# facebookresearch/metamorph

Measured on AMD Instinct MI355X. Metric: train tokens/sec (LLaMA-3-8B + SigLIP-SO400M, seq2048, 256 img toks), whole job, higher is better.
Workload: dtype bf16

## Files before the change

metamorph_amd/csrc/attn.hip:

```cpp
#include "mm355_common.h"
#include "attn2.h"
#include <cstdlib>
#include <algorithm>

namespace {

constexpr int NT = 256;

__global__ __launch_bounds__(NT) void attn_delta_kernel(const uint16_t* __restrict__ o, const uint16_t* __restrict__ d_o, int64_t ld_o,
                                                        float* __restrict__ delta, int L, int Hq, int d) {
    const int l = blockIdx.x * 64 + (threadIdx.x >> 2), part = threadIdx.x & 3;
    const int h = blockIdx.y, b = blockIdx.z;
    const int dv = d >> 3;
    float s = 0.f;
    if (l < L) {
        for (int v = part; v < dv; v += 4) {
            float x[8], y[8];
            unpack8(*(const u32x4*)(o + ((int64_t)b * L + l) * ld_o + (int64_t)h * d + v * 8), x);
            unpack8(*(const u32x4*)(d_o + ((int64_t)b * L + l) * ld_o + (int64_t)h * d + v * 8), y);
#pragma unroll
            for (int e = 0; e < 8; ++e) s += x[e] * y[e];
        }
    }
    s += __shfl_xor(s, 1, 64);
    s += __shfl_xor(s, 2, 64);
    if (part == 0 && l < L) delta[((int64_t)b * Hq + h) * L + l] = s;
}

__global__ __launch_bounds__(NT) void group_reduce_kernel(const float* __restrict__ part, uint16_t* __restrict__ out, int64_t ld_out, int64_t rows,
                                                          int Hq, int Hkv, int d) {
    const int group = Hq / Hkv, cv = (Hkv * d) >> 3;
    const int64_t total = rows * cv;
    for (int64_t i = blockIdx.x * (int64_t)NT + threadIdx.x; i < total; i += (int64_t)gridDim.x * NT) {
        const int64_t r = i / cv; const int c = (int)(i % cv) * 8;
        const int hk = c / d, cc = c % d;
        float acc[8] = {0.f, 0.f, 0.f, 0.f, 0.f, 0.f, 0.f, 0.f};
        for (int g = 0; g < group; ++g) {
            const float* p = part + r * ((int64_t)Hq * d) + (int64_t)(hk * group + g) * d + cc;
            const f32x4 x0 = *(const f32x4*)p, x1 = *(const f32x4*)(p + 4);
            acc[0] += x0.x; acc[1] += x0.y; acc[2] += x0.z; acc[3] += x0.w;
            acc[4] += x1.x; acc[5] += x1.y; acc[6] += x1.z; acc[7] += x1.w;
        }
        *(u32x4*)(out + r * ld_out + c) = pack8(acc);
    }
}

int pick_dp(int64_t d) { return d <= 64 ? 64 : (d <= 96 ? 96 : 128); }

bool bad_geom(int64_t B, int64_t L, int64_t Hq, int64_t Hkv, int64_t d) {
    return B <= 0 || L <= 0 || Hq <= 0 || Hkv <= 0 || (Hq % Hkv) || d <= 0 || d > 128 || (d & 7) || L > 0x7fffffff;
}

bool fast128(int64_t d, int64_t ld_k) { return d == 128 && ld_k * 2 * 64 < 0x7fffffff; }

}

namespace {
int attn_fwd_impl(const mm355_bf16* q, const mm355_bf16* k, const mm355_bf16* v, int64_t ld_q, int64_t ld_k, mm355_bf16* o,
                  int64_t ld_o, float* lse, const int32_t* seqlens, int64_t B, int64_t L, int64_t Hq, int64_t Hkv,
                  int64_t d, float scale, int causal, int variant, void* stream, int32_t* dbg = nullptr) {
    (void)hipGetLastError();
    if (!q || !k || !v || !o || !lse || bad_geom(B, L, Hq, Hkv, d)) return MM355_EINVAL;
    if ((ld_q & 7) || (ld_k & 7) || (ld_o & 7)) return MM355_EINVAL;
    attn2::Args a{q, k, v, nullptr, ld_q, ld_k, ld_o, o, lse, nullptr, nullptr, nullptr, 0, seqlens,
                  nullptr, nullptr, nullptr, nullptr, 0, (int)B, (int)L, (int)Hq, (int)Hkv, (int)d, scale, causal, nullptr, nullptr, nullptr, dbg};
    const bool can4 = d == 128 && L * ld_k * 2 < 0x7fffffffll;
    if (variant == 4 || variant == 41) return can4 ? mm355_attn4_fwd_launch(a, variant == 41, (hipStream_t)stream) : MM355_EUNSUPPORTED;
    if (variant == 3) return MM355_EUNSUPPORTED;
    if (variant == 2) return mm355_attn2_fwd_launch(a, pick_dp(d), (hipStream_t)stream);
    if (variant != 0) return MM355_EINVAL;
    if (can4 && fast128(d, ld_k)) return mm355_attn4_fwd_launch(a, 0, (hipStream_t)stream);
    return mm355_attn2_fwd_launch(a, pick_dp(d), (hipStream_t)stream);
}
}

extern "C" int mm355_attn_fwd(const mm355_bf16* q, const mm355_bf16* k, const mm355_bf16* v, int64_t ld_q, int64_t ld_k, mm355_bf16* o,
                              int64_t ld_o, float* lse, const int32_t* seqlens, int64_t B, int64_t L, int64_t Hq, int64_t Hkv,
                              int64_t d, float scale, int causal, void* stream) {
    return attn_fwd_impl(q, k, v, ld_q, ld_k, o, ld_o, lse, seqlens, B, L, Hq, Hkv, d, scale, causal, 0, stream);
}

extern "C" int mm355_attn_fwd_variant(const mm355_bf16* q, const mm355_bf16* k, const mm355_bf16* v, int64_t ld_q, int64_t ld_k, mm355_bf16* o,
                                      int64_t ld_o, float* lse, const int32_t* seqlens, int64_t B, int64_t L, int64_t Hq, int64_t Hkv,
                                      int64_t d, float scale, int causal, int variant, void* stream) {
    return attn_fwd_impl(q, k, v, ld_q, ld_k, o, ld_o, lse, seqlens, B, L, Hq, Hkv, d, scale, causal, variant, stream);
}

extern "C" int mm355_attn_fwd_debug(const mm355_bf16* q, const mm355_bf16* k, const mm355_bf16* v, int64_t ld_q, int64_t ld_k, mm355_bf16* o,
                                    int64_t ld_o, float* lse, const int32_t* seqlens, int64_t B, int64_t L, int64_t Hq, int64_t Hkv,
                                    int64_t d, float scale, int causal, int variant, int32_t* rescale_counts, void* stream) {
    if (!rescale_counts || (variant != 4 && variant != 41)) return MM355_EINVAL;
    return attn_fwd_impl(q, k, v, ld_q, ld_k, o, ld_o, lse, seqlens, B, L, Hq, Hkv, d, scale, causal, variant, stream, rescale_counts);
}

extern "C" int mm355_attn_bwd_prep(const mm355_bf16* o, const mm355_bf16* d_o, int64_t ld_o, float* delta, int64_t B, int64_t L,
                                   int64_t Hq, int64_t d, void* stream) {
    (void)hipGetLastError();
    if (!o || !d_o || !delta || B <= 0 || L <= 0 || Hq <= 0 || d <= 0 || d > 128 || (d & 7) || (ld_o & 7)) return MM355_EINVAL;
    dim3 grid((unsigned)((L + 63) / 64), (unsigned)Hq, (unsigned)B);
    hipLaunchKernelGGL(attn_delta_kernel, grid, dim3(NT), 0, (hipStream_t)stream, o, d_o, ld_o, delta, (int)L, (int)Hq, (int)d);
    return mm_launch_status();
}

extern "C" int64_t mm355_attn_bwd_ws_floats(int64_t B, int64_t L, int64_t Hq, int64_t Hkv, int64_t d, int64_t ld_max) {
    if (fast128(d, ld_max)) return 2 * B * Hq * L;
    if (Hq == Hkv) return 0;
    return 2 * B * L * Hq * d;
}

namespace {
int attn_bwd_impl(const mm355_bf16* q, const mm355_bf16* k, const mm355_bf16* v, int64_t ld_q, int64_t ld_k, const mm355_bf16* d_o,
                  int64_t ld_o, const float* lse, const float* delta, const int32_t* seqlens, mm355_bf16* dq, int64_t ld_dq,
                  mm355_bf16* dk, mm355_bf16* dv, int64_t ld_dkv, int64_t B, int64_t L, int64_t Hq, int64_t Hkv, int64_t d,
                  float scale, int causal, float* workspace, const uint16_t* rope_cos, const uint16_t* rope_sin, const int32_t* rope_pos,
                  int variant, void* stream) {
    (void)hipGetLastError();
    if (!q || !k || !v || !d_o || !lse || !delta || !dq || !dk || !dv || bad_geom(B, L, Hq, Hkv, d)) return MM355_EINVAL;
    if ((ld_q & 7) || (ld_k & 7) || (ld_o & 7) || (ld_dkv & 7) || (ld_dq & 7)) return MM355_EINVAL;
    const int64_t ld_max = std::max(std::max(ld_q, ld_k), ld_o);
    if (variant == 3) return MM355_EUNSUPPORTED;
    if (variant != 0 && variant != 2 && variant != 4 && variant != 41) return MM355_EINVAL;
    const bool is128 = fast128(d, ld_max) && variant != 2;
    const bool can4 = is128 && workspace && L * ld_max * 2 < 0x7fffffffll;
    if (is128 && !can4 && Hq != Hkv) return workspace ? MM355_EUNSUPPORTED : MM355_EINVAL;
    if (rope_cos && !can4) return MM355_EUNSUPPORTED;
    if ((variant == 4 || variant == 41) && !can4) return MM355_EUNSUPPORTED;
    if (variant == 4 || variant == 41 || (variant == 0 && can4)) {
        attn2::Args a4{q, k, v, d_o, ld_q, ld_k, ld_o, nullptr, nullptr, lse, delta, dq, ld_dq, seqlens,
                       dk, dv, nullptr, nullptr, ld_dkv, (int)B, (int)L, (int)Hq, (int)Hkv, (int)d, scale, causal, rope_cos, rope_sin, rope_pos};
        return mm355_attn4_bwd_launch(a4, workspace, variant == 41, (hipStream_t)stream);
    }
    if (Hq != Hkv && !workspace) return MM355_EINVAL;
    hipStream_t s = (hipStream_t)stream;
    float* dkp = nullptr;
    float* dvp = nullptr;
    if (Hq != Hkv) {
        dkp = workspace;
        dvp = workspace + (int64_t)B * L * Hq * d;
    }
    attn2::Args a{q, k, v, d_o, ld_q, ld_k, ld_o, nullptr, nullptr, lse, delta, dq, ld_dq, seqlens,
                  dk, dv, dkp, dvp, ld_dkv, (int)B, (int)L, (int)Hq, (int)Hkv, (int)d, scale, causal, rope_cos, rope_sin, rope_pos};
    int rc = mm355_attn2_dkdv_launch(a, pick_dp(d), s);
    if (rc != MM355_OK) return rc;
    if (dkp) {
        const int64_t rows = B * L;
        const unsigned rg = (unsigned)std::min<int64_t>((rows * (Hkv * d / 8) + NT - 1) / NT, 4096);
        hipLaunchKernelGGL(group_reduce_kernel, dim3(rg), dim3(NT), 0, s, dkp, dk, ld_dkv, rows, (int)Hq, (int)Hkv, (int)d);
        hipLaunchKernelGGL(group_reduce_kernel, dim3(rg), dim3(NT), 0, s, dvp, dv, ld_dkv, rows, (int)Hq, (int)Hkv, (int)d);
        rc = mm_launch_status();
        if (rc != MM355_OK) return rc;
    }
    return mm355_attn2_dq_launch(a, pick_dp(d), s);
}
}

extern "C" int mm355_attn_bwd(const mm355_bf16* q, const mm355_bf16* k, const mm355_bf16* v, int64_t ld_q, int64_t ld_k, const mm355_bf16* d_o,
                              int64_t ld_o, const float* lse, const float* delta, const int32_t* seqlens, mm355_bf16* dq, int64_t ld_dq,
                              mm355_bf16* dk, mm355_bf16* dv, int64_t ld_dkv, int64_t B, int64_t L, int64_t Hq, int64_t Hkv, int64_t d,
                              float scale, int causal, float* workspace, void* stream) {
    return attn_bwd_impl(q, k, v, ld_q, ld_k, d_o, ld_o, lse, delta, seqlens, dq, ld_dq, dk, dv, ld_dkv, B, L, Hq, Hkv, d, scale, causal, workspace,
                         nullptr, nullptr, nullptr, 0, stream);
}

extern "C" int mm355_attn_bwd_rope(const mm355_bf16* q, const mm355_bf16* k, const mm355_bf16* v, int64_t ld_q, int64_t ld_k, const mm355_bf16* d_o,
                                   int64_t ld_o, const float* lse, const float* delta, const int32_t* seqlens, mm355_bf16* dq, int64_t ld_dq,
                                   mm355_bf16* dk, mm355_bf16* dv, int64_t ld_dkv, int64_t B, int64_t L, int64_t Hq, int64_t Hkv, int64_t d,
                                   float scale, int causal, const mm355_bf16* cos_t, const mm355_bf16* sin_t, const int32_t* pos_offset,
                                   float* workspace, void* stream) {
    if (!cos_t || !sin_t) return MM355_EINVAL;
    return attn_bwd_impl(q, k, v, ld_q, ld_k, d_o, ld_o, lse, delta, seqlens, dq, ld_dq, dk, dv, ld_dkv, B, L, Hq, Hkv, d, scale, causal, workspace,
                         cos_t, sin_t, pos_offset, 0, stream);
}

extern "C" int mm355_attn_bwd_variant(const mm355_bf16* q, const mm355_bf16* k, const mm355_bf16* v, int64_t ld_q, int64_t ld_k, const mm355_bf16* d_o,
                                      int64_t ld_o, const float* lse, const float* delta, const int32_t* seqlens, mm355_bf16* dq, int64_t ld_dq,
                                      mm355_bf16* dk, mm355_bf16* dv, int64_t ld_dkv, int64_t B, int64_t L, int64_t Hq, int64_t Hkv, int64_t d,
                                      float scale, int causal, const mm355_bf16* cos_t, const mm355_bf16* sin_t, const int32_t* pos_offset,
                                      float* workspace, int variant, void* stream) {
    if ((cos_t == nullptr) != (sin_t == nullptr)) return MM355_EINVAL;
    return attn_bwd_impl(q, k, v, ld_q, ld_k, d_o, ld_o, lse, delta, seqlens, dq, ld_dq, dk, dv, ld_dkv, B, L, Hq, Hkv, d, scale, causal, workspace,
                         cos_t, sin_t, pos_offset, variant, stream);
}
```

metamorph_amd/csrc/attn4.hip:

```cpp
#include "attn2.h"

#ifndef ATTN4_GEN_DIR
#define ATTN4_GEN_DIR attn4_gen
#endif
#define ATTN4_STR2(x) #x
#define ATTN4_STR(x) ATTN4_STR2(x)
#define ATTN4_INC(f) ATTN4_STR(ATTN4_GEN_DIR/f)

namespace attn4 {
using namespace attn2;

constexpr int TILE = 16384;
constexpr int VRING = 2 * TILE;
constexpr float LOG2E = 1.4426950408889634f;
constexpr float THR = 6.0f;

MM_DEV float half_swap_max(float m) {
    float a = m, b = m;
    asm volatile("" : "+v"(b));
    swap32(a, b);
    return max2_raw(a, b);
}
MM_DEV float half_swap_sum(float m) {
    float a = m, b = m;
    asm volatile("" : "+v"(b));
    swap32(a, b);
    return a + b;
}

#define ATTN4_BARRIER() do { if (do_bar) asm volatile("s_waitcnt vmcnt(0)\n\ts_barrier" ::: "memory"); } while (0)
#define ATTN4_DMA_K(i) do { __builtin_amdgcn_sched_barrier(0); \
    __builtin_amdgcn_raw_ptr_buffer_load_lds(rsK, (lptr_t)(smem + kdst + (i) * 1024), 16, kvo[i], 0, 0, 0); __builtin_amdgcn_sched_barrier(0); } while (0)
#define ATTN4_DMA_V(i) do { if (do_bar) { __builtin_amdgcn_sched_barrier(0); \
    __builtin_amdgcn_raw_ptr_buffer_load_lds(rsV, (lptr_t)(smem + vdst + (i) * 1024), 16, vvo[i], 0, 0, 0); __builtin_amdgcn_sched_barrier(0); } } while (0)
template <bool SAFE>
__global__ __launch_bounds__(256, 1) __attribute__((amdgpu_num_vgpr(64))) void fwd_kernel(Args a) {
    __shared__ __attribute__((aligned(16))) unsigned char smem[4 * TILE];
    asm volatile("" ::: "v255", "a255");
#ifdef MM355_ATTN4_TIMING
    const long long tm0 = __builtin_readcyclecounter();
    long long tm1 = 0, tm2 = 0, tm3 = 0, tm4 = 0, tm5 = 0;
#define ATTN4_STAMP(x) x = __builtin_readcyclecounter()
#else
#define ATTN4_STAMP(x) do {} while (0)
#endif
    const int tid = threadIdx.x, lane = tid & 63;
    const int wave = __builtin_amdgcn_readfirstlane(tid >> 6);
    const int c = lane & 31, hi = lane >> 5;
    int xb, hq, b;
    block_coords((a.L + 255) / 256, a.Hq, inner_heads(a.Hq, a.Hq / a.Hkv), true, xb, hq, b);
    const int q0 = xb * 256;
    const int hk = hq / (a.Hq / a.Hkv);
    const int L = a.L;
    const int seqlen = a.seqlens ? min(a.seqlens[b], L) : L;
    const int64_t row_base = (int64_t)b * L;
    uint16_t* o_base = a.o + row_base * a.ld_o + (int64_t)hq * 128;
    float* lse_base = a.lse + ((int64_t)b * a.Hq + hq) * L;

    if (q0 >= seqlen) {
        for (int v = tid; v < 256 * 16; v += 256) {
            const int r = v >> 4, cc = (v & 15) * 8;
            if (q0 + r < L) *(u32x4*)(o_base + (int64_t)(q0 + r) * a.ld_o + cc) = u32x4{0u, 0u, 0u, 0u};
        }
        if (q0 + tid < L) lse_base[q0 + tid] = 0.f;
        return;
    }
    const int kv_end = a.causal ? min(seqlen, q0 + 256) : seqlen;
    const int T = (kv_end + 63) >> 6;
    const int qw0 = q0 + wave * 64;
    const int tw = qw0 < seqlen ? (a.causal ? min(T - 1, min(qw0 + 63, seqlen - 1) >> 6) : T - 1) : -1;

    const uint32_t ldb = (uint32_t)a.ld_k * 2u;
    const uint16_t* kbase = a.k + row_base * a.ld_k + (int64_t)hk * 128;
    const uint16_t* vbase = a.v + row_base * a.ld_k + (int64_t)hk * 128;
    const uint32_t nrec = (uint32_t)(seqlen - 1) * ldb + 256u;
    __amdgpu_buffer_rsrc_t rsK, rsV;
#define ATTN4_TILE_RSRC(base_, tile_) __builtin_amdgcn_make_buffer_rsrc((void*)((base_) + (int64_t)(tile_) * 64 * a.ld_k), 0, \
    (tile_) < T ? nrec - (uint32_t)(tile_) * 64u * ldb : 0u, 0x00020000)
    uint32_t kvo[4], vvo[4];
    {
        const int r4 = lane >> 4, pc = lane & 15;
#pragma unroll
        for (int i = 0; i < 4; ++i) {
            const uint32_t row = 16 * wave + 4 * i + r4;
            kvo[i] = row * ldb + (uint32_t)((pc ^ (4 * i + r4)) << 4);
            vvo[i] = row * ldb + (uint32_t)((pc ^ (r4 << 2)) << 4);
        }
    }
    const float sl2 = a.scale * LOG2E;
    const uint32_t sl2b_ = __builtin_amdgcn_readfirstlane(__float_as_uint(sl2));
    {
        const uint16_t* qp0_ = a.q + (row_base + min(qw0 + c, L - 1)) * a.ld_q + (int64_t)hq * 128 + hi * 8;
        const uint16_t* qp1_ = a.q + (row_base + min(qw0 + 32 + c, L - 1)) * a.ld_q + (int64_t)hq * 128 + hi * 8;
#include ATTN4_INC(q_load.inc)
    }
    bool do_bar = true;
    int kdst, vdst;
    rsK = ATTN4_TILE_RSRC(kbase, 0); rsV = ATTN4_TILE_RSRC(vbase, 0); kdst = wave * 4096; vdst = VRING + wave * 4096;
#pragma unroll
    for (int i = 0; i < 4; ++i) { ATTN4_DMA_K(i); }
#pragma unroll
    for (int i = 0; i < 4; ++i) { ATTN4_DMA_V(i); }
    rsK = ATTN4_TILE_RSRC(kbase, 1); kdst = TILE + wave * 4096;
#pragma unroll
    for (int i = 0; i < 4; ++i) { ATTN4_DMA_K(i); }
#include ATTN4_INC(zero_o.inc)
    float LS[2][4] = {{0.f, 0.f, 0.f, 0.f}, {0.f, 0.f, 0.f, 0.f}};
    float MX[2][2], rm_[2], rt_[2];
    uint64_t grow_ = 0;
    int nresc_ = 0;
#define ATTN4_COUNT_RESCALE() (++nresc_)
    float thr_ = THR / sl2;
    asm volatile("" : "+v"(thr_));
    const float ninf = -INFINITY;
    int KA[8], VA[4];
#pragma unroll
    for (int ks = 0; ks < 8; ++ks) KA[ks] = c * 256 + (((ks * 2 + hi) ^ (c & 15)) << 4);
    {
        const int g = lane >> 4, i = lane & 15;
#pragma unroll
        for (int db = 0; db < 4; ++db)
            VA[db] = VRING + (4 * hi + (i >> 2)) * 256 + ((((db * 4 + (g & 1) * 2 + ((i & 3) >> 1)) ^ ((i >> 2) << 2))) << 4) + (i & 1) * 8;
    }
#pragma unroll
    for (int ks = 0; ks < 8; ++ks) asm volatile("" : "+v"(KA[ks]));
#pragma unroll
    for (int i = 0; i < 4; ++i) { asm volatile("" : "+v"(VA[i])); asm volatile("" : "+v"(kvo[i])); asm volatile("" : "+v"(vvo[i])); }
    int lim2[2] = {0, 0};
    if (tw >= 0) {
#pragma unroll
        for (int qb = 0; qb < 2; ++qb) {
            const int qg = qw0 + qb * 32 + c;
            lim2[qb] = (a.causal ? min(qg, seqlen - 1) : seqlen - 1) - tw * 64 - 4 * hi;
        }
    }
    asm volatile("s_waitcnt vmcnt(12)" ::: "memory");
#include ATTN4_INC(q_pre01.inc)
    asm volatile("s_waitcnt vmcnt(0)" ::: "memory");
    __builtin_amdgcn_s_barrier();

#define ATTN4_STEP_VARS(s_) do { const int s__ = (s_); \
    rsK = ATTN4_TILE_RSRC(kbase, s__ + 2); rsV = ATTN4_TILE_RSRC(vbase, s__ + 2); \
    kdst = (s__ & 1) * TILE + wave * 4096; vdst = VRING + (s__ & 1) * TILE + wave * 4096; } while (0)

    ATTN4_STAMP(tm1);
    if (tw >= 0) {
        bool mask_next = tw == 0;
        ATTN4_STEP_VARS(-1);
        if constexpr (SAFE) {
#include ATTN4_INC(safe_head.inc)
        } else {
#include ATTN4_INC(head.inc)
        }
        ATTN4_STAMP(tm2);
        int t = 0;
        for (;;) {
            if (t >= tw) break;
            mask_next = t + 1 == tw;
            ATTN4_STEP_VARS(t);
            if constexpr (SAFE) {
#include ATTN4_INC(safe_loop0.inc)
            } else {
#include ATTN4_INC(loop0.inc)
            }
            ++t;
            if (t >= tw) break;
            mask_next = t + 1 == tw;
            ATTN4_STEP_VARS(t);
            if constexpr (SAFE) {
#include ATTN4_INC(safe_loop1.inc)
            } else {
#include ATTN4_INC(loop1.inc)
            }
            ++t;
        }
        ATTN4_STAMP(tm3);
        do_bar = tw <= T - 2;
        ATTN4_STEP_VARS(tw);
        if (tw & 1) {
            if constexpr (SAFE) {
#include ATTN4_INC(safe_tail1.inc)
            } else {
#include ATTN4_INC(tail1.inc)
            }
        } else {
            if constexpr (SAFE) {
#include ATTN4_INC(safe_tail0.inc)
            } else {
#include ATTN4_INC(tail0.inc)
            }
        }
    }
    ATTN4_STAMP(tm4);
    do_bar = true;
    for (int s = tw < 0 ? -1 : tw + 1; s <= T - 2; ++s) {
        ATTN4_STEP_VARS(s);
        if (s >= 0) {
#pragma unroll
            for (int i = 0; i < 4; ++i) { ATTN4_DMA_K(i); }
        }
        ATTN4_BARRIER();
#pragma unroll
        for (int i = 0; i < 4; ++i) { ATTN4_DMA_V(i); }
    }
    asm volatile("s_nop 15\n\ts_nop 15\n\ts_nop 15\n\ts_nop 15\n\ts_waitcnt vmcnt(0) lgkmcnt(0)" ::: "memory");
    __syncthreads();
    ATTN4_STAMP(tm5);

    unsigned char* so = smem + wave * TILE;
#pragma unroll
    for (int qb_ = 0; qb_ < 2; ++qb_) {
        const int qg = qw0 + qb_ * 32 + c;
        const bool valid = qg < seqlen && tw >= 0;
        const float l_run = half_swap_sum((LS[qb_][0] + LS[qb_][1]) + (LS[qb_][2] + LS[qb_][3]));
        const float inv = (valid && l_run > 0.f) ? 1.0f / l_run : 0.f;
#pragma unroll
        for (int db_ = 0; db_ < 4; ++db_) {
            float x_[16];
#include ATTN4_INC(epi_read.inc)
#pragma unroll
            for (int i4 = 0; i4 < 4; ++i4) {
                u32x2 w;
                w.x = pack2bf(x_[4 * i4 + 0] * inv, x_[4 * i4 + 1] * inv);
                w.y = pack2bf(x_[4 * i4 + 2] * inv, x_[4 * i4 + 3] * inv);
                *(u32x2*)(so + (qb_ * 32 + c) * 256 + (((db_ * 4 + i4) ^ (c & 15)) << 4) + hi * 8) = w;
            }
        }
        float nm0;
        if (qb_ == 0) asm volatile("v_mov_b32 %0, v192" : "=v"(nm0)); else asm volatile("v_mov_b32 %0, v208" : "=v"(nm0));
        if (hi == 0 && qg < L) lse_base[qg] = valid ? (log2f(l_run) - nm0 * sl2) * 0.6931471805599453f : 0.f;
    }
    __syncthreads();
#pragma unroll
    for (int k = 0; k < 16; ++k) {
        const int r = 4 * k + (lane >> 4), j = lane & 15;
        const int qg = qw0 + r;
        if (qg < L) *(u32x4*)(o_base + (int64_t)qg * a.ld_o + j * 8) = *(const u32x4*)(so + r * 256 + ((j ^ (r & 15)) << 4));
    }
    if (a.dbg && lane == 0) a.dbg[(((int64_t)b * a.Hq + hq) * ((L + 255) / 256) + xb) * 4 + wave] = nresc_;
#ifdef MM355_ATTN4_TIMING
    asm volatile("s_waitcnt vmcnt(0)" ::: "memory");
    const long long tm6 = __builtin_readcyclecounter();
    if (lane == 0 && (wave == 0 || wave == 3) && q0 + 64 <= L) {
        long long* w = (long long*)(lse_base + q0) + (wave == 3 ? 8 : 0);
        w[0] = tm1 - tm0; w[1] = tm2 - tm1; w[2] = tm3 - tm2; w[3] = tm4 - tm3; w[4] = tm5 - tm4; w[5] = tm6 - tm5; w[6] = tw; w[7] = T;
    }
#endif
}

}

int mm355_attn4_fwd_launch(const attn2::Args& a, int variant, hipStream_t s) {
    const int64_t nblk = (int64_t)((a.L + 255) / 256) * a.Hq * a.B;
    if (nblk > 0x7fffffff) return MM355_EINVAL;
    if (variant == 1) hipLaunchKernelGGL(attn4::fwd_kernel<true>, dim3((unsigned)nblk), dim3(256), 0, s, a);
    else hipLaunchKernelGGL(attn4::fwd_kernel<false>, dim3((unsigned)nblk), dim3(256), 0, s, a);
    return mm_launch_status();
}
```

metamorph_amd/csrc/attn4_bwd.hip:

```cpp
#include "attn2.h"

#ifndef ATTN4B_GEN_DIR
#define ATTN4B_GEN_DIR attn4_bwd_gen
#endif
#define ATTN4B_STR2(x) #x
#define ATTN4B_STR(x) ATTN4B_STR2(x)
#define ATTN4B_INC(f) ATTN4B_STR(ATTN4B_GEN_DIR/f)

namespace attn4b {
using namespace attn2;

constexpr float LOG2E = 1.4426950408889634f;
constexpr int SLOT = 32768;
constexpr int KV_BASE = 2048;
constexpr int KV_LDS = KV_BASE + 4 * SLOT, Q_LDS = 4 * SLOT;

MM_DEV int rot4(int row) { return ((row & 3) << 2) | ((row >> 2) & 3); }

struct LaneAddr {
    int RA[8], TA[4], TB[4], SA;
    MM_DEV void init(int lane) {
        const int c = lane & 31, hi = lane >> 5, g = lane >> 4, i = lane & 15;
#pragma unroll
        for (int ks = 0; ks < 8; ++ks) RA[ks] = c * 256 + (((ks * 2 + hi) ^ rot4(c)) << 4);
        const int row0 = 4 * hi + (i >> 2), row1 = row0 + 8;
#pragma unroll
        for (int db = 0; db < 4; ++db) {
            const int chunk = db * 4 + (g & 1) * 2 + ((i & 3) >> 1);
            TA[db] = row0 * 256 + ((chunk ^ rot4(row0)) << 4) + (i & 1) * 8;
            TB[db] = row1 * 256 + ((chunk ^ rot4(row1)) << 4) + (i & 1) * 8;
        }
        SA = hi * 16;
    }
};
MM_DEV void piece_offsets(int wave, int lane, uint32_t ldb, uint32_t (&vo)[4]) {
    const int r4 = lane >> 4, pc = lane & 15;
#pragma unroll
    for (int i = 0; i < 4; ++i) vo[i] = (uint32_t)(16 * wave + 4 * i + r4) * ldb + (uint32_t)((pc ^ ((r4 << 2) | i)) << 4);
}
MM_DEV uint32_t scale_pair(uint32_t w, float s) { return pack2bf(bflo(w) * s, bfhi(w) * s); }

#define BWD_BARRIER() asm volatile("s_waitcnt vmcnt(%0)\n\ts_barrier" :: "n"(NDMA) : "memory")

template <bool SAFE>
__global__ __launch_bounds__(256, 1) __attribute__((amdgpu_num_vgpr(96))) void dkdv_kernel(Args a, const float* __restrict__ nstat) {
    extern __shared__ __attribute__((aligned(16))) unsigned char smem[];
    asm volatile("" ::: "v255", "a255");
#ifdef MM355_ATTN4_TIMING
    const long long tm0 = __builtin_readcyclecounter();
    long long tm1 = 0, tm2 = 0, tm3 = 0, tm4 = 0;
#define BWD_STAMP(x) x = __builtin_readcyclecounter()
#else
#define BWD_STAMP(x) do {} while (0)
#endif
    constexpr int NDMA = 9;
    const int tid = threadIdx.x, lane = tid & 63;
    const int wave = __builtin_amdgcn_readfirstlane(tid >> 6);
    const int c = lane & 31, hi = lane >> 5;
    const int rep = a.Hq / a.Hkv;
    int xb, hk, b;
    block_coords((a.L + 127) / 128, a.Hkv, inner_heads(a.Hkv, 1), false, xb, hk, b);
    const int kv0 = xb * 128;
    const int L = a.L;
    const int seqlen = a.seqlens ? min(a.seqlens[b], L) : L;
    const int64_t row_base = (int64_t)b * L;
    const int kw0 = kv0 + 32 * wave;

    if (kv0 >= seqlen) {
        for (int v = tid; v < 128 * 16; v += 256) {
            const int r = v >> 4, cc = (v & 15) * 8;
            if (kv0 + r < L) {
                *(u32x4*)(a.dk + (row_base + kv0 + r) * a.ld_dkv + (int64_t)hk * 128 + cc) = u32x4{0u, 0u, 0u, 0u};
                *(u32x4*)(a.dv + (row_base + kv0 + r) * a.ld_dkv + (int64_t)hk * 128 + cc) = u32x4{0u, 0u, 0u, 0u};
            }
        }
        return;
    }
    const int q_start = a.causal ? kv0 : 0;
    const int n_it = (seqlen - q_start + 63) >> 6;
    const int n_tot = n_it * rep;
    const uint32_t ldqb = (uint32_t)a.ld_q * 2u, ldob = (uint32_t)a.ld_o * 2u;
    const int64_t stat_n = (int64_t)a.B * a.Hq * L;

    const uint32_t sl2b_ = __builtin_amdgcn_readfirstlane(__float_as_uint(a.scale * LOG2E));
    LaneAddr la;
    la.init(lane);
    int RA[8], TA[4], TB[4], RAH[8], TAH[4], TBH[4], SA = la.SA;
#pragma unroll
    for (int i = 0; i < 8; ++i) { RA[i] = la.RA[i] + KV_BASE; RAH[i] = RA[i] + 65536; asm volatile("" : "+v"(RA[i])); asm volatile("" : "+v"(RAH[i])); }
#pragma unroll
    for (int i = 0; i < 4; ++i) {
        TA[i] = la.TA[i] + KV_BASE; TB[i] = la.TB[i] + KV_BASE; TAH[i] = TA[i] + 65536; TBH[i] = TB[i] + 65536;
        asm volatile("" : "+v"(TA[i])); asm volatile("" : "+v"(TB[i])); asm volatile("" : "+v"(TAH[i])); asm volatile("" : "+v"(TBH[i]));
    }
    asm volatile("" : "+v"(SA));
    uint32_t qvo[4], ovo[4], svo = (uint32_t)lane * 4u;
    piece_offsets(wave, lane, ldqb, qvo);
    piece_offsets(wave, lane, ldob, ovo);
#pragma unroll
    for (int i = 0; i < 4; ++i) { asm volatile("" : "+v"(qvo[i])); asm volatile("" : "+v"(ovo[i])); }
    asm volatile("" : "+v"(svo));
    const float ninf = -INFINITY;
    float t0_;
    const int kg = kw0 + c;
    const int qmin = kg >= seqlen ? seqlen : (a.causal ? kg : 0);
    const int mlo_base = qmin - 4 * hi;
    const unsigned mspan_ = (unsigned)(seqlen - qmin);
    int mlo_ = 0;
    bool mask_cur = false;

    __amdgpu_buffer_rsrc_t rsQ, rsO, rsS;
    int dst0 = 0;
    int dg = 0, dit = 0, cg = 0, cit = 0;
#define KV_TILE_VARS(slot_) do { \
        const bool live_ = dg < rep; \
        const int qt0_ = q_start + dit * 64; \
        const int hq_ = hk * rep + dg; \
        rsQ = __builtin_amdgcn_make_buffer_rsrc((void*)(a.q + (row_base + qt0_) * a.ld_q + (int64_t)hq_ * 128), 0, live_ ? (uint32_t)(seqlen - qt0_ - 1) * ldqb + 256u : 0u, 0x00020000); \
        rsO = __builtin_amdgcn_make_buffer_rsrc((void*)(a.d_o + (row_base + qt0_) * a.ld_o + (int64_t)hq_ * 128), 0, live_ ? (uint32_t)(seqlen - qt0_ - 1) * ldob + 256u : 0u, 0x00020000); \
        rsS = __builtin_amdgcn_make_buffer_rsrc((void*)(nstat + (wave & 1) * stat_n + ((int64_t)b * a.Hq + hq_) * L + qt0_), 0, live_ ? (uint32_t)(L - qt0_) * 4u : 0u, 0x00020000); \
        dst0 = (slot_); \
        if (++dit == n_it) { dit = 0; ++dg; } } while (0)
#define BWD_DMA(i) do { __builtin_amdgcn_sched_barrier(0); \
        if ((i) < 4) __builtin_amdgcn_raw_ptr_buffer_load_lds(rsQ, (lptr_t)(smem + KV_BASE + dst0 * SLOT + (wave * 4 + (i)) * 1024), 16, qvo[(i) & 3], 0, 0, 0); \
        else if ((i) < 8) __builtin_amdgcn_raw_ptr_buffer_load_lds(rsO, (lptr_t)(smem + KV_BASE + dst0 * SLOT + 16384 + (wave * 4 + (i) - 4) * 1024), 16, ovo[(i) & 3], 0, 0, 0); \
        else __builtin_amdgcn_raw_ptr_buffer_load_lds(rsS, (lptr_t)(smem + dst0 * 512 + (wave & 1) * 256), 4, svo, 0, 0, 0); \
        __builtin_amdgcn_sched_barrier(0); } while (0)
#define KV_MASK_VARS() do { \
        const int qt0_ = q_start + cit * 64; \
        mask_cur = (a.causal && qt0_ < kw0 + 31) || qt0_ + 64 > seqlen || kw0 + 32 > seqlen; \
        mlo_ = mlo_base - qt0_; \
        if (++cit == n_it) { cit = 0; ++cg; } } while (0)

    KV_TILE_VARS(0);
#pragma unroll
    for (int i = 0; i < 9; ++i) { BWD_DMA(i); }
    KV_TILE_VARS(1);
#pragma unroll
    for (int i = 0; i < 9; ++i) { BWD_DMA(i); }
    {
        const int key = min(kw0 + c, L - 1);
        const uint16_t* p0_ = a.k + (row_base + key) * a.ld_k + (int64_t)hk * 128 + hi * 8;
        const uint16_t* p1_ = a.v + (row_base + key) * a.ld_k + (int64_t)hk * 128 + hi * 8;
#include ATTN4B_INC(kv_pers_load.inc)
    }
#include ATTN4B_INC(kv_zero.inc)
    asm volatile("s_waitcnt vmcnt(0)" ::: "memory");
    {
        float t1_;
#include ATTN4B_INC(kv_pers_place.inc)
    }
    __builtin_amdgcn_s_barrier();

    BWD_STAMP(tm1);
    KV_TILE_VARS(2);
    if constexpr (SAFE) {
#include ATTN4B_INC(kv_safe_head.inc)
    } else {
#include ATTN4B_INC(kv_head.inc)
    }
    BWD_STAMP(tm2);
    int u = 0;
    for (;;) {
        if (u >= n_tot - 1) break;
        KV_TILE_VARS(3); KV_MASK_VARS();
        if constexpr (SAFE) {
#include ATTN4B_INC(kv_safe_loop0.inc)
        } else {
#include ATTN4B_INC(kv_loop0.inc)
        }
        ++u;
        if (u >= n_tot - 1) break;
        KV_TILE_VARS(0); KV_MASK_VARS();
        if constexpr (SAFE) {
#include ATTN4B_INC(kv_safe_loop1.inc)
        } else {
#include ATTN4B_INC(kv_loop1.inc)
        }
        ++u;
        if (u >= n_tot - 1) break;
        KV_TILE_VARS(1); KV_MASK_VARS();
        if constexpr (SAFE) {
#include ATTN4B_INC(kv_safe_loop2.inc)
        } else {
#include ATTN4B_INC(kv_loop2.inc)
        }
        ++u;
        if (u >= n_tot - 1) break;
        KV_TILE_VARS(2); KV_MASK_VARS();
        if constexpr (SAFE) {
#include ATTN4B_INC(kv_safe_loop3.inc)
        } else {
#include ATTN4B_INC(kv_loop3.inc)
        }
        ++u;
    }
    BWD_STAMP(tm3);
    KV_MASK_VARS();
    switch (u & 3) {
    case 0:
        if constexpr (SAFE) {
#include ATTN4B_INC(kv_safe_tail0.inc)
        } else {
#include ATTN4B_INC(kv_tail0.inc)
        }
        break;
    case 1:
        if constexpr (SAFE) {
#include ATTN4B_INC(kv_safe_tail1.inc)
        } else {
#include ATTN4B_INC(kv_tail1.inc)
        }
        break;
    case 2:
        if constexpr (SAFE) {
#include ATTN4B_INC(kv_safe_tail2.inc)
        } else {
#include ATTN4B_INC(kv_tail2.inc)
        }
        break;
    default:
        if constexpr (SAFE) {
#include ATTN4B_INC(kv_safe_tail3.inc)
        } else {
#include ATTN4B_INC(kv_tail3.inc)
        }
        break;
    }
#undef BWD_DMA
    asm volatile("s_nop 15\n\ts_nop 15\n\ts_nop 15\n\ts_nop 15\n\ts_waitcnt vmcnt(0) lgkmcnt(0)" ::: "memory");
    __syncthreads();
    BWD_STAMP(tm4);

    unsigned char* so = smem + wave * 16384;
    const int pos = min(kg, L - 1) + (a.rope_pos ? a.rope_pos[b] : 0);
#pragma unroll
    for (int which_ = 0; which_ < 2; ++which_) {
        const float sc = which_ == 0 ? a.scale : 1.0f;
#pragma unroll
        for (int dbp = 0; dbp < 2; ++dbp)
#pragma unroll
            for (int i4_ = 0; i4_ < 4; ++i4_) {
                float x_[4], lo_[4], hi_[4];
                {
                    const int db_ = dbp;
#include ATTN4B_INC(kv_acc_read.inc)
#pragma unroll
                    for (int r = 0; r < 4; ++r) lo_[r] = x_[r] * sc;
                }
                {
                    const int db_ = dbp + 2;
#include ATTN4B_INC(kv_acc_read.inc)
#pragma unroll
                    for (int r = 0; r < 4; ++r) hi_[r] = x_[r] * sc;
                }
                if (which_ == 0 && a.rope_cos) {
                    const int col = dbp * 32 + 8 * i4_ + 4 * hi;
                    const u32x2 cw = *(const u32x2*)(a.rope_cos + (int64_t)pos * 128 + col);
                    const u32x2 sw = *(const u32x2*)(a.rope_sin + (int64_t)pos * 128 + col);
                    const float cs[4] = {bflo(cw.x), bfhi(cw.x), bflo(cw.y), bfhi(cw.y)};
                    const float sn[4] = {bflo(sw.x), bfhi(sw.x), bflo(sw.y), bfhi(sw.y)};
#pragma unroll
                    for (int r = 0; r < 4; ++r) {
                        const float x1 = round_bf(lo_[r]), x2 = round_bf(hi_[r]);
                        lo_[r] = x1 * cs[r] + x2 * sn[r];
                        hi_[r] = x2 * cs[r] - x1 * sn[r];
                    }
                }
#pragma unroll
                for (int half = 0; half < 2; ++half) {
                    const int db = dbp + 2 * half;
                    const float* s4 = half ? hi_ : lo_;
                    u32x2 w;
                    w.x = pack2bf(s4[0], s4[1]);
                    w.y = pack2bf(s4[2], s4[3]);
                    *(u32x2*)(so + which_ * 8192 + c * 256 + (((db * 4 + i4_) ^ (c & 15)) << 4) + hi * 8) = w;
                }
            }
    }
    __syncthreads();
#pragma unroll
    for (int which_ = 0; which_ < 2; ++which_)
#pragma unroll
        for (int k = 0; k < 8; ++k) {
            const int r = 4 * k + (lane >> 4), j = lane & 15;
            const int key = kw0 + r;
            if (key < L) {
                u32x4 val = *(const u32x4*)(so + which_ * 8192 + r * 256 + ((j ^ (r & 15)) << 4));
                if (key >= seqlen) val = u32x4{0u, 0u, 0u, 0u};
                *(u32x4*)((which_ ? a.dv : a.dk) + (row_base + key) * a.ld_dkv + (int64_t)hk * 128 + j * 8) = val;
            }
        }
#ifdef MM355_ATTN4_TIMING
    asm volatile("s_waitcnt vmcnt(0)" ::: "memory");
    const long long tm5 = __builtin_readcyclecounter();
    __syncthreads();
    if (tid == 0) {
        long long* w = (long long*)(a.dk + (row_base + kv0) * a.ld_dkv + (int64_t)hk * 128);
        w[0] = tm1 - tm0; w[1] = tm2 - tm1; w[2] = tm3 - tm2; w[3] = tm4 - tm3; w[4] = tm5 - tm4; w[5] = n_tot;
    }
#endif
}

template <bool SAFE>
__global__ __launch_bounds__(256, 1) __attribute__((amdgpu_num_vgpr(80))) void dq_kernel(Args a) {
    extern __shared__ __attribute__((aligned(16))) unsigned char smem[];
    asm volatile("" ::: "v255", "a255");
    constexpr int NDMA = 8;
    const int tid = threadIdx.x, lane = tid & 63;
    const int wave = __builtin_amdgcn_readfirstlane(tid >> 6);
    const int c = lane & 31, hi = lane >> 5;
    int xb, hq, b;
    block_coords((a.L + 127) / 128, a.Hq, inner_heads(a.Hq, a.Hq / a.Hkv), true, xb, hq, b);
    const int q0 = xb * 128;
    const int hk = hq / (a.Hq / a.Hkv);
    const int L = a.L;
    const int seqlen = a.seqlens ? min(a.seqlens[b], L) : L;
    const int64_t row_base = (int64_t)b * L;
    uint16_t* dq_base = a.dqb + row_base * a.ld_dq + (int64_t)hq * 128;
    if (q0 >= seqlen) {
        for (int v = tid; v < 128 * 16; v += 256) {
            const int r = v >> 4, cc = (v & 15) * 8;
            if (q0 + r < L) *(u32x4*)(dq_base + (int64_t)(q0 + r) * a.ld_dq + cc) = u32x4{0u, 0u, 0u, 0u};
        }
        return;
    }
    const int kv_end = a.causal ? min(seqlen, q0 + 128) : seqlen;
    const int n_tot = (kv_end + 63) >> 6;
    const int qw0 = q0 + 32 * wave;
    const int qg = qw0 + c;
    const uint32_t ldb = (uint32_t)a.ld_k * 2u;
    const uint16_t* kbase = a.k + row_base * a.ld_k + (int64_t)hk * 128;
    const uint16_t* vbase = a.v + row_base * a.ld_k + (int64_t)hk * 128;
    const uint32_t nrec = (uint32_t)(seqlen - 1) * ldb + 256u;

    const uint32_t sl2b_ = __builtin_amdgcn_readfirstlane(__float_as_uint(a.scale * LOG2E));
    LaneAddr la;
    la.init(lane);
    int RA[8], TA[4], TB[4], RAH[8], TAH[4], TBH[4];
#pragma unroll
    for (int i = 0; i < 8; ++i) { RA[i] = la.RA[i]; RAH[i] = RA[i] + 65536; asm volatile("" : "+v"(RA[i])); asm volatile("" : "+v"(RAH[i])); }
#pragma unroll
    for (int i = 0; i < 4; ++i) {
        TA[i] = la.TA[i]; TB[i] = la.TB[i]; TAH[i] = TA[i] + 65536; TBH[i] = TB[i] + 65536;
        asm volatile("" : "+v"(TA[i])); asm volatile("" : "+v"(TB[i])); asm volatile("" : "+v"(TAH[i])); asm volatile("" : "+v"(TBH[i]));
    }
    uint32_t kvo[4];
    piece_offsets(wave, lane, ldb, kvo);
#pragma unroll
    for (int i = 0; i < 4; ++i) asm volatile("" : "+v"(kvo[i]));
    const float ninf = -INFINITY;
    const int kmax = qg >= seqlen ? -1 : (a.causal ? min(qg, seqlen - 1) : seqlen - 1);
    const int mlim_base = kmax - 4 * hi;
    int mlim_ = 0;
    bool mask_cur = false;

    __amdgpu_buffer_rsrc_t rsK, rsV;
    int dst0 = 0, dt = 0, ct = 0;
#define Q_TILE_VARS(slot_) do { \
        rsK = __builtin_amdgcn_make_buffer_rsrc((void*)(kbase + (int64_t)dt * 64 * a.ld_k), 0, dt < n_tot ? nrec - (uint32_t)dt * 64u * ldb : 0u, 0x00020000); \
        rsV = __builtin_amdgcn_make_buffer_rsrc((void*)(vbase + (int64_t)dt * 64 * a.ld_k), 0, dt < n_tot ? nrec - (uint32_t)dt * 64u * ldb : 0u, 0x00020000); \
        dst0 = (slot_) * SLOT; ++dt; } while (0)
#define BWD_DMA(i) do { __builtin_amdgcn_sched_barrier(0); \
        if ((i) < 4) __builtin_amdgcn_raw_ptr_buffer_load_lds(rsK, (lptr_t)(smem + dst0 + (wave * 4 + (i)) * 1024), 16, kvo[(i) & 3], 0, 0, 0); \
        else __builtin_amdgcn_raw_ptr_buffer_load_lds(rsV, (lptr_t)(smem + dst0 + 16384 + (wave * 4 + (i) - 4) * 1024), 16, kvo[(i) & 3], 0, 0, 0); \
        __builtin_amdgcn_sched_barrier(0); } while (0)
#define Q_MASK_VARS() do { \
        const int kt0_ = ct * 64; \
        mask_cur = (a.causal && kt0_ + 63 > qw0) || kt0_ + 64 > seqlen || qw0 + 32 > seqlen; \
        mlim_ = mlim_base - kt0_; ++ct; } while (0)

    Q_TILE_VARS(0);
#pragma unroll
    for (int i = 0; i < 8; ++i) { BWD_DMA(i); }
    Q_TILE_VARS(1);
#pragma unroll
    for (int i = 0; i < 8; ++i) { BWD_DMA(i); }
    {
        const int qc = min(qg, L - 1);
        const uint16_t* p0_ = a.q + (row_base + qc) * a.ld_q + (int64_t)hq * 128 + hi * 8;
        const uint16_t* p1_ = a.d_o + (row_base + qc) * a.ld_o + (int64_t)hq * 128 + hi * 8;
#include ATTN4B_INC(q_pers_load.inc)
        const float nl_ = -a.lse_in[((int64_t)b * a.Hq + hq) * L + qc] * (1.0f / a.scale);
        const float nd_ = -a.delta[((int64_t)b * a.Hq + hq) * L + qc];
#include ATTN4B_INC(q_tuple_write.inc)
    }
#include ATTN4B_INC(q_zero.inc)
    asm volatile("s_waitcnt vmcnt(0)" ::: "memory");
    {
        float t0_, t1_;
#include ATTN4B_INC(q_pers_place.inc)
    }
    __builtin_amdgcn_s_barrier();

    Q_TILE_VARS(2);
    if constexpr (SAFE) {
#include ATTN4B_INC(q_safe_head.inc)
    } else {
#include ATTN4B_INC(q_head.inc)
    }
    int u = 0;
    for (;;) {
        if (u >= n_tot - 1) break;
        Q_TILE_VARS(3); Q_MASK_VARS();
        if constexpr (SAFE) {
#include ATTN4B_INC(q_safe_loop0.inc)
        } else {
#include ATTN4B_INC(q_loop0.inc)
        }
        ++u;
        if (u >= n_tot - 1) break;
        Q_TILE_VARS(0); Q_MASK_VARS();
        if constexpr (SAFE) {
#include ATTN4B_INC(q_safe_loop1.inc)
        } else {
#include ATTN4B_INC(q_loop1.inc)
        }
        ++u;
        if (u >= n_tot - 1) break;
        Q_TILE_VARS(1); Q_MASK_VARS();
        if constexpr (SAFE) {
#include ATTN4B_INC(q_safe_loop2.inc)
        } else {
#include ATTN4B_INC(q_loop2.inc)
        }
        ++u;
        if (u >= n_tot - 1) break;
        Q_TILE_VARS(2); Q_MASK_VARS();
        if constexpr (SAFE) {
#include ATTN4B_INC(q_safe_loop3.inc)
        } else {
#include ATTN4B_INC(q_loop3.inc)
        }
        ++u;
    }
    Q_MASK_VARS();
    switch (u & 3) {
    case 0:
        if constexpr (SAFE) {
#include ATTN4B_INC(q_safe_tail0.inc)
        } else {
#include ATTN4B_INC(q_tail0.inc)
        }
        break;
    case 1:
        if constexpr (SAFE) {
#include ATTN4B_INC(q_safe_tail1.inc)
        } else {
#include ATTN4B_INC(q_tail1.inc)
        }
        break;
    case 2:
        if constexpr (SAFE) {
#include ATTN4B_INC(q_safe_tail2.inc)
        } else {
#include ATTN4B_INC(q_tail2.inc)
        }
        break;
    default:
        if constexpr (SAFE) {
#include ATTN4B_INC(q_safe_tail3.inc)
        } else {
#include ATTN4B_INC(q_tail3.inc)
        }
        break;
    }
#undef BWD_DMA
    asm volatile("s_nop 15\n\ts_nop 15\n\ts_nop 15\n\ts_nop 15\n\ts_waitcnt vmcnt(0) lgkmcnt(0)" ::: "memory");
    __syncthreads();

    unsigned char* so = smem + wave * 8192;
    const float keep = qg < seqlen ? a.scale : 0.0f;
    const int pos = min(qg, L - 1) + (a.rope_pos ? a.rope_pos[b] : 0);
#pragma unroll
    for (int dbp = 0; dbp < 2; ++dbp)
#pragma unroll
        for (int i4_ = 0; i4_ < 4; ++i4_) {
            constexpr int which_ = 0;
            float x_[4], lo_[4], hi_[4];
            {
                const int db_ = dbp;
#include ATTN4B_INC(q_acc_read.inc)
#pragma unroll
                for (int r = 0; r < 4; ++r) lo_[r] = x_[r] * keep;
            }
            {
                const int db_ = dbp + 2;
#include ATTN4B_INC(q_acc_read.inc)
#pragma unroll
                for (int r = 0; r < 4; ++r) hi_[r] = x_[r] * keep;
            }
            if (a.rope_cos) {
                const int col = dbp * 32 + 8 * i4_ + 4 * hi;
                const u32x2 cw = *(const u32x2*)(a.rope_cos + (int64_t)pos * 128 + col);
                const u32x2 sw = *(const u32x2*)(a.rope_sin + (int64_t)pos * 128 + col);
                const float cs[4] = {bflo(cw.x), bfhi(cw.x), bflo(cw.y), bfhi(cw.y)};
                const float sn[4] = {bflo(sw.x), bfhi(sw.x), bflo(sw.y), bfhi(sw.y)};
#pragma unroll
                for (int r = 0; r < 4; ++r) {
                    const float x1 = round_bf(lo_[r]), x2 = round_bf(hi_[r]);
                    lo_[r] = x1 * cs[r] + x2 * sn[r];
                    hi_[r] = x2 * cs[r] - x1 * sn[r];
                }
            }
#pragma unroll
            for (int half = 0; half < 2; ++half) {
                const int db = dbp + 2 * half;
                const float* s4 = half ? hi_ : lo_;
                u32x2 w;
                w.x = pack2bf(s4[0], s4[1]);
                w.y = pack2bf(s4[2], s4[3]);
                *(u32x2*)(so + c * 256 + (((db * 4 + i4_) ^ (c & 15)) << 4) + hi * 8) = w;
            }
        }
    __syncthreads();
#pragma unroll
    for (int k = 0; k < 8; ++k) {
        const int r = 4 * k + (lane >> 4), j = lane & 15;
        if (qw0 + r < L) *(u32x4*)(dq_base + (int64_t)(qw0 + r) * a.ld_dq + j * 8) = *(const u32x4*)(so + r * 256 + ((j ^ (r & 15)) << 4));
    }
}

__global__ __launch_bounds__(256) void nstat_kernel(const float* __restrict__ lse, const float* __restrict__ delta, float* __restrict__ nstat, int64_t n,
                                                    float inv_scale) {
    for (int64_t i = blockIdx.x * 256ll + threadIdx.x; i < n; i += (int64_t)gridDim.x * 256) {
        nstat[i] = -lse[i] * inv_scale;
        nstat[n + i] = -delta[i];
    }
}

}

int mm355_attn4_bwd_launch(const attn2::Args& a, float* workspace, int variant, hipStream_t s) {
    static std::atomic<uint64_t> ok_kv{0}, ok_kvs{0}, ok_q{0}, ok_qs{0};
    const int64_t n = (int64_t)a.B * a.Hq * a.L;
    hipLaunchKernelGGL(attn4b::nstat_kernel, dim3((unsigned)std::min<int64_t>((n + 255) / 256, 2048)), dim3(256), 0, s, a.lse_in, a.delta, workspace, n, 1.0f / a.scale);
    const int64_t nkv = (int64_t)((a.L + 127) / 128) * a.Hkv * a.B, nq = (int64_t)((a.L + 127) / 128) * a.Hq * a.B;
    if (nkv > 0x7fffffff || nq > 0x7fffffff) return MM355_EINVAL;
    if (variant == 1) {
        if (mm_ensure_dynamic_lds((const void*)attn4b::dkdv_kernel<true>, attn4b::KV_LDS, ok_kvs) != MM355_OK) return MM355_ELAUNCH;
        if (mm_ensure_dynamic_lds((const void*)attn4b::dq_kernel<true>, attn4b::Q_LDS, ok_qs) != MM355_OK) return MM355_ELAUNCH;
        hipLaunchKernelGGL(attn4b::dkdv_kernel<true>, dim3((unsigned)nkv), dim3(256), attn4b::KV_LDS, s, a, (const float*)workspace);
        hipLaunchKernelGGL(attn4b::dq_kernel<true>, dim3((unsigned)nq), dim3(256), attn4b::Q_LDS, s, a);
    } else {
        if (mm_ensure_dynamic_lds((const void*)attn4b::dkdv_kernel<false>, attn4b::KV_LDS, ok_kv) != MM355_OK) return MM355_ELAUNCH;
        if (mm_ensure_dynamic_lds((const void*)attn4b::dq_kernel<false>, attn4b::Q_LDS, ok_q) != MM355_OK) return MM355_ELAUNCH;
        hipLaunchKernelGGL(attn4b::dkdv_kernel<false>, dim3((unsigned)nkv), dim3(256), attn4b::KV_LDS, s, a, (const float*)workspace);
        hipLaunchKernelGGL(attn4b::dq_kernel<false>, dim3((unsigned)nq), dim3(256), attn4b::Q_LDS, s, a);
    }
    return mm_launch_status();
}
```

Baseline: 25740.

## Pair causal query blocks per workgroup in attn4 forward and dq kernels

For causal attention, each workgroup in the attn4 forward and dq-backward kernels now handles two query blocks, a late one and an early one (nb-1-xb and xb). This balances the triangular workload across workgroups and halves the grid. It also prefetches the next block's Q and K/V while the current block's epilogue runs, using a larger dynamic LDS region so the output staging buffer is separate. New variant codes (41-45) select the pairing and safe modes. The cost is a more complex kernel with more register pressure and extra LDS.

Result: no change. 25650 (-0.3%).

```diff
diff --git a/metamorph_amd/csrc/attn.hip b/metamorph_amd/csrc/attn.hip
--- a/metamorph_amd/csrc/attn.hip
+++ b/metamorph_amd/csrc/attn.hip
@@ -53,6 +53,8 @@
 
 bool fast128(int64_t d, int64_t ld_k) { return d == 128 && ld_k * 2 * 64 < 0x7fffffff; }
 
+int stream_variant(int variant) { return variant == 4 ? 0 : (variant >= 41 && variant <= 45 ? variant - 40 : -1); }
+
 }
 
 namespace {
@@ -65,7 +67,7 @@
     attn2::Args a{q, k, v, nullptr, ld_q, ld_k, ld_o, o, lse, nullptr, nullptr, nullptr, 0, seqlens,
                   nullptr, nullptr, nullptr, nullptr, 0, (int)B, (int)L, (int)Hq, (int)Hkv, (int)d, scale, causal, nullptr, nullptr, nullptr, dbg};
     const bool can4 = d == 128 && L * ld_k * 2 < 0x7fffffffll;
-    if (variant == 4 || variant == 41) return can4 ? mm355_attn4_fwd_launch(a, variant == 41, (hipStream_t)stream) : MM355_EUNSUPPORTED;
+    if (stream_variant(variant) >= 0) return can4 ? mm355_attn4_fwd_launch(a, stream_variant(variant), (hipStream_t)stream) : MM355_EUNSUPPORTED;
     if (variant == 3) return MM355_EUNSUPPORTED;
     if (variant == 2) return mm355_attn2_fwd_launch(a, pick_dp(d), (hipStream_t)stream);
     if (variant != 0) return MM355_EINVAL;
@@ -89,7 +91,7 @@
 extern "C" int mm355_attn_fwd_debug(const mm355_bf16* q, const mm355_bf16* k, const mm355_bf16* v, int64_t ld_q, int64_t ld_k, mm355_bf16* o,
                                     int64_t ld_o, float* lse, const int32_t* seqlens, int64_t B, int64_t L, int64_t Hq, int64_t Hkv,
                                     int64_t d, float scale, int causal, int variant, int32_t* rescale_counts, void* stream) {
-    if (!rescale_counts || (variant != 4 && variant != 41)) return MM355_EINVAL;
+    if (!rescale_counts || stream_variant(variant) < 0) return MM355_EINVAL;
     return attn_fwd_impl(q, k, v, ld_q, ld_k, o, ld_o, lse, seqlens, B, L, Hq, Hkv, d, scale, causal, variant, stream, rescale_counts);
 }
 
@@ -119,16 +121,17 @@
     if ((ld_q & 7) || (ld_k & 7) || (ld_o & 7) || (ld_dkv & 7) || (ld_dq & 7)) return MM355_EINVAL;
     const int64_t ld_max = std::max(std::max(ld_q, ld_k), ld_o);
     if (variant == 3) return MM355_EUNSUPPORTED;
-    if (variant != 0 && variant != 2 && variant != 4 && variant != 41) return MM355_EINVAL;
+    const int sv = stream_variant(variant);
+    if (variant != 0 && variant != 2 && sv < 0) return MM355_EINVAL;
     const bool is128 = fast128(d, ld_max) && variant != 2;
     const bool can4 = is128 && workspace && L * ld_max * 2 < 0x7fffffffll;
     if (is128 && !can4 && Hq != Hkv) return workspace ? MM355_EUNSUPPORTED : MM355_EINVAL;
     if (rope_cos && !can4) return MM355_EUNSUPPORTED;
-    if ((variant == 4 || variant == 41) && !can4) return MM355_EUNSUPPORTED;
-    if (variant == 4 || variant == 41 || (variant == 0 && can4)) {
+    if (sv >= 0 && !can4) return MM355_EUNSUPPORTED;
+    if (sv >= 0 || (variant == 0 && can4)) {
         attn2::Args a4{q, k, v, d_o, ld_q, ld_k, ld_o, nullptr, nullptr, lse, delta, dq, ld_dq, seqlens,
                        dk, dv, nullptr, nullptr, ld_dkv, (int)B, (int)L, (int)Hq, (int)Hkv, (int)d, scale, causal, rope_cos, rope_sin, rope_pos};
-        return mm355_attn4_bwd_launch(a4, workspace, variant == 41, (hipStream_t)stream);
+        return mm355_attn4_bwd_launch(a4, workspace, sv >= 0 ? sv : 0, (hipStream_t)stream);
     }
     if (Hq != Hkv && !workspace) return MM355_EINVAL;
     hipStream_t s = (hipStream_t)stream;
diff --git a/metamorph_amd/csrc/attn4.hip b/metamorph_amd/csrc/attn4.hip
--- a/metamorph_amd/csrc/attn4.hip
+++ b/metamorph_amd/csrc/attn4.hip
@@ -33,12 +33,16 @@
     __builtin_amdgcn_raw_ptr_buffer_load_lds(rsK, (lptr_t)(smem + kdst + (i) * 1024), 16, kvo[i], 0, 0, 0); __builtin_amdgcn_sched_barrier(0); } while (0)
 #define ATTN4_DMA_V(i) do { if (do_bar) { __builtin_amdgcn_sched_barrier(0); \
     __builtin_amdgcn_raw_ptr_buffer_load_lds(rsV, (lptr_t)(smem + vdst + (i) * 1024), 16, vvo[i], 0, 0, 0); __builtin_amdgcn_sched_barrier(0); } } while (0)
+constexpr int STAGE = 4 * TILE, FWD_LDS = 8 * TILE;
+MM_DEV void q_load(const uint16_t* qp0_, const uint16_t* qp1_) {
+#include ATTN4_INC(q_load.inc)
+}
 template <bool SAFE>
-__global__ __launch_bounds__(256, 1) __attribute__((amdgpu_num_vgpr(64))) void fwd_kernel(Args a) {
-    __shared__ __attribute__((aligned(16))) unsigned char smem[4 * TILE];
+__global__ __launch_bounds__(256, 1) __attribute__((amdgpu_num_vgpr(64))) void fwd_kernel(Args a, int paired) {
+    extern __shared__ __attribute__((aligned(16))) unsigned char smem[];
     asm volatile("" ::: "v255", "a255");
 #ifdef MM355_ATTN4_TIMING
-    const long long tm0 = __builtin_readcyclecounter();
+    long long tm0 = __builtin_readcyclecounter();
     long long tm1 = 0, tm2 = 0, tm3 = 0, tm4 = 0, tm5 = 0;
 #define ATTN4_STAMP(x) x = __builtin_readcyclecounter()
 #else
@@ -46,10 +50,9 @@
 #endif
     const int tid = threadIdx.x, lane = tid & 63;
     const int wave = __builtin_amdgcn_readfirstlane(tid >> 6);
-    const int c = lane & 31, hi = lane >> 5;
+    const int nb = (a.L + 255) / 256;
     int xb, hq, b;
-    block_coords((a.L + 255) / 256, a.Hq, inner_heads(a.Hq, a.Hq / a.Hkv), true, xb, hq, b);
-    const int q0 = xb * 256;
+    block_coords(paired ? (nb + 1) / 2 : nb, a.Hq, inner_heads(a.Hq, a.Hq / a.Hkv), true, xb, hq, b);
     const int hk = hq / (a.Hq / a.Hkv);
     const int L = a.L;
     const int seqlen = a.seqlens ? min(a.seqlens[b], L) : L;
@@ -57,18 +60,17 @@
     uint16_t* o_base = a.o + row_base * a.ld_o + (int64_t)hq * 128;
     float* lse_base = a.lse + ((int64_t)b * a.Hq + hq) * L;
 
-    if (q0 >= seqlen) {
+    int q0 = (paired ? nb - 1 - xb : xb) * 256;
+    int q0n = (paired && nb - 1 - xb != xb) ? xb * 256 : -1;
+    while (q0 >= seqlen) {
         for (int v = tid; v < 256 * 16; v += 256) {
             const int r = v >> 4, cc = (v & 15) * 8;
             if (q0 + r < L) *(u32x4*)(o_base + (int64_t)(q0 + r) * a.ld_o + cc) = u32x4{0u, 0u, 0u, 0u};
         }
         if (q0 + tid < L) lse_base[q0 + tid] = 0.f;
-        return;
+        if (q0n < 0) return;
+        q0 = q0n; q0n = -1;
     }
-    const int kv_end = a.causal ? min(seqlen, q0 + 256) : seqlen;
-    const int T = (kv_end + 63) >> 6;
-    const int qw0 = q0 + wave * 64;
-    const int tw = qw0 < seqlen ? (a.causal ? min(T - 1, min(qw0 + 63, seqlen - 1) >> 6) : T - 1) : -1;
 
     const uint32_t ldb = (uint32_t)a.ld_k * 2u;
     const uint16_t* kbase = a.k + row_base * a.ld_k + (int64_t)hk * 128;
@@ -77,183 +79,223 @@
     __amdgpu_buffer_rsrc_t rsK, rsV;
 #define ATTN4_TILE_RSRC(base_, tile_) __builtin_amdgcn_make_buffer_rsrc((void*)((base_) + (int64_t)(tile_) * 64 * a.ld_k), 0, \
     (tile_) < T ? nrec - (uint32_t)(tile_) * 64u * ldb : 0u, 0x00020000)
-    uint32_t kvo[4], vvo[4];
-    {
-        const int r4 = lane >> 4, pc = lane & 15;
-#pragma unroll
-        for (int i = 0; i < 4; ++i) {
-            const uint32_t row = 16 * wave + 4 * i + r4;
-            kvo[i] = row * ldb + (uint32_t)((pc ^ (4 * i + r4)) << 4);
-            vvo[i] = row * ldb + (uint32_t)((pc ^ (r4 << 2)) << 4);
-        }
-    }
     const float sl2 = a.scale * LOG2E;
     const uint32_t sl2b_ = __builtin_amdgcn_readfirstlane(__float_as_uint(sl2));
-    {
-        const uint16_t* qp0_ = a.q + (row_base + min(qw0 + c, L - 1)) * a.ld_q + (int64_t)hq * 128 + hi * 8;
-        const uint16_t* qp1_ = a.q + (row_base + min(qw0 + 32 + c, L - 1)) * a.ld_q + (int64_t)hq * 128 + hi * 8;
-#include ATTN4_INC(q_load.inc)
-    }
-    bool do_bar = true;
-    int kdst, vdst;
-    rsK = ATTN4_TILE_RSRC(kbase, 0); rsV = ATTN4_TILE_RSRC(vbase, 0); kdst = wave * 4096; vdst = VRING + wave * 4096;
-#pragma unroll
-    for (int i = 0; i < 4; ++i) { ATTN4_DMA_K(i); }
-#pragma unroll
-    for (int i = 0; i < 4; ++i) { ATTN4_DMA_V(i); }
-    rsK = ATTN4_TILE_RSRC(kbase, 1); kdst = TILE + wave * 4096;
-#pragma unroll
-    for (int i = 0; i < 4; ++i) { ATTN4_DMA_K(i); }
-#include ATTN4_INC(zero_o.inc)
-    float LS[2][4] = {{0.f, 0.f, 0.f, 0.f}, {0.f, 0.f, 0.f, 0.f}};
-    float MX[2][2], rm_[2], rt_[2];
-    uint64_t grow_ = 0;
-    int nresc_ = 0;
-#define ATTN4_COUNT_RESCALE() (++nresc_)
     float thr_ = THR / sl2;
     asm volatile("" : "+v"(thr_));
     const float ninf = -INFINITY;
-    int KA[8], VA[4];
-#pragma unroll
-    for (int ks = 0; ks < 8; ++ks) KA[ks] = c * 256 + (((ks * 2 + hi) ^ (c & 15)) << 4);
-    {
-        const int g = lane >> 4, i = lane & 15;
-#pragma unroll
-        for (int db = 0; db < 4; ++db)
-            VA[db] = VRING + (4 * hi + (i >> 2)) * 256 + ((((db * 4 + (g & 1) * 2 + ((i & 3) >> 1)) ^ ((i >> 2) << 2))) << 4) + (i & 1) * 8;
+    int qb0 = 0, T = 0, qw0 = 0, tw = 0;
+    int lim2[2] = {0, 0};
+    bool do_bar = true, seam = false;
+    int kdst, vdst;
+#define ATTN4_PIECE_OFFSETS(lane_) do { \
+        const int r4 = (lane_) >> 4, pc = (lane_) & 15; \
+        _Pragma("unroll") for (int i = 0; i < 4; ++i) { \
+            const uint32_t row = 16 * wave + 4 * i + r4; \
+            kvo[i] = row * ldb + (uint32_t)((pc ^ (4 * i + r4)) << 4); \
+            vvo[i] = row * ldb + (uint32_t)((pc ^ (r4 << 2)) << 4); \
+        } } while (0)
+#define ATTN4_BLOCK_ISSUE(q0_) do { \
+        qb0 = (q0_); \
+        int li_ = lane; \
+        asm volatile("" : "+v"(li_)); \
+        const int c_ = li_ & 31, hi_ = li_ >> 5; \
+        const int kv_end_ = a.causal ? min(seqlen, qb0 + 256) : seqlen; \
+        T = (kv_end_ + 63) >> 6; \
+        qw0 = qb0 + wave * 64; \
+        tw = qw0 < seqlen ? (a.causal ? min(T - 1, min(qw0 + 63, seqlen - 1) >> 6) : T - 1) : -1; \
+        lim2[0] = lim2[1] = 0; \
+        if (tw >= 0) { \
+            _Pragma("unroll") for (int qb = 0; qb < 2; ++qb) { \
+                const int qg = qw0 + qb * 32 + c_; \
+                lim2[qb] = (a.causal ? min(qg, seqlen - 1) : seqlen - 1) - tw * 64 - 4 * hi_; \
+            } \
+        } \
+        const uint16_t* qp0_ = a.q + (row_base + min(qw0 + c_, L - 1)) * a.ld_q + (int64_t)hq * 128 + hi_ * 8; \
+        const uint16_t* qp1_ = a.q + (row_base + min(qw0 + 32 + c_, L - 1)) * a.ld_q + (int64_t)hq * 128 + hi_ * 8; \
+        q_load(qp0_, qp1_); \
+        uint32_t kvo[4], vvo[4]; \
+        ATTN4_PIECE_OFFSETS(li_); \
+        do_bar = true; \
+        rsK = ATTN4_TILE_RSRC(kbase, 0); rsV = ATTN4_TILE_RSRC(vbase, 0); kdst = wave * 4096; vdst = VRING + wave * 4096; \
+        _Pragma("unroll") for (int i = 0; i < 4; ++i) { ATTN4_DMA_K(i); } \
+        _Pragma("unroll") for (int i = 0; i < 4; ++i) { ATTN4_DMA_V(i); } \
+        rsK = ATTN4_TILE_RSRC(kbase, 1); kdst = TILE + wave * 4096; \
+        _Pragma("unroll") for (int i = 0; i < 4; ++i) { ATTN4_DMA_K(i); } } while (0)
+
+    ATTN4_BLOCK_ISSUE(q0);
+    for (;;) {
+        int ln_ = lane;
+        asm volatile("" : "+v"(ln_));
+        uint32_t kvo[4], vvo[4];
+        ATTN4_PIECE_OFFSETS(ln_);
+#include ATTN4_INC(zero_o.inc)
+        float LS[2][4] = {{0.f, 0.f, 0.f, 0.f}, {0.f, 0.f, 0.f, 0.f}};
+        float MX[2][2], rm_[2], rt_[2];
+        uint64_t grow_ = 0;
+        int nresc_ = 0;
+#define ATTN4_COUNT_RESCALE() (++nresc_)
+        int KA[8], VA[4];
+        {
+            const int c = ln_ & 31, hi = ln_ >> 5;
+#pragma unroll
+            for (int ks = 0; ks < 8; ++ks) KA[ks] = c * 256 + (((ks * 2 + hi) ^ (c & 15)) << 4);
+            const int g = ln_ >> 4, i = ln_ & 15;
+#pragma unroll
+            for (int db = 0; db < 4; ++db)
+                VA[db] = VRING + (4 * hi + (i >> 2)) * 256 + ((((db * 4 + (g & 1) * 2 + ((i & 3) >> 1)) ^ ((i >> 2) << 2))) << 4) + (i & 1) * 8;
+        }
+#pragma unroll
+        for (int ks = 0; ks < 8; ++ks) asm volatile("" : "+v"(KA[ks]));
+#pragma unroll
+        for (int i = 0; i < 4; ++i) { asm volatile("" : "+v"(VA[i])); asm volatile("" : "+v"(kvo[i])); asm volatile("" : "+v"(vvo[i])); }
+        if (seam) asm volatile("s_waitcnt vmcnt(0)" ::: "memory");
+        else asm volatile("s_waitcnt vmcnt(12)" ::: "memory");
+#include ATTN4_INC(q_pre01.inc)
+        asm volatile("s_waitcnt vmcnt(0)" ::: "memory");
+        __builtin_amdgcn_s_barrier();
+
+#define ATTN4_STEP_VARS(s_) do { const int s__ = (s_); \
+        rsK = ATTN4_TILE_RSRC(kbase, s__ + 2); rsV = ATTN4_TILE_RSRC(vbase, s__ + 2); \
+        kdst = (s__ & 1) * TILE + wave * 4096; vdst = VRING + (s__ & 1) * TILE + wave * 4096; } while (0)
+
+        ATTN4_STAMP(tm1);
+        if (tw >= 0) {
+            bool mask_next = tw == 0;
+            ATTN4_STEP_VARS(-1);
+            if constexpr (SAFE) {
+#include ATTN4_INC(safe_head.inc)
+            } else {
+#include ATTN4_INC(head.inc)
+            }
+            ATTN4_STAMP(tm2);
+            int t = 0;
+            for (;;) {
+                if (t >= tw) break;
+                mask_next = t + 1 == tw;
+                ATTN4_STEP_VARS(t);
+                if constexpr (SAFE) {
+#include ATTN4_INC(safe_loop0.inc)
+                } else {
+#include ATTN4_INC(loop0.inc)
+                }
+                ++t;
+                if (t >= tw) break;
+                mask_next = t + 1 == tw;
+                ATTN4_STEP_VARS(t);
+                if constexpr (SAFE) {
+#include ATTN4_INC(safe_loop1.inc)
+                } else {
+#include ATTN4_INC(loop1.inc)
+                }
+                ++t;
+            }
+            ATTN4_STAMP(tm3);
+            do_bar = tw <= T - 2;
+            ATTN4_STEP_VARS(tw);
+            if (tw & 1) {
+                if constexpr (SAFE) {
+#include ATTN4_INC(safe_tail1.inc)
+                } else {
+#include ATTN4_INC(tail1.inc)
+                }
+            } else {
+                if constexpr (SAFE) {
+#include ATTN4_INC(safe_tail0.inc)
+                } else {
+#include ATTN4_INC(tail0.inc)
+                }
+            }
+        }
+        ATTN4_STAMP(tm4);
+        do_bar = true;
+        for (int s = tw < 0 ? -1 : tw + 1; s <= T - 2; ++s) {
+            ATTN4_STEP_VARS(s);
+            if (s >= 0) {
+#pragma unroll
+                for (int i = 0; i < 4; ++i) { ATTN4_DMA_K(i); }
+            }
+            ATTN4_BARRIER();
+#pragma unroll
+            for (int i = 0; i < 4; ++i) { ATTN4_DMA_V(i); }
+        }
+        asm volatile("s_nop 15\n\ts_nop 15\n\ts_nop 15\n\ts_nop 15\n\ts_waitcnt vmcnt(0) lgkmcnt(0)" ::: "memory");
+        __syncthreads();
+        ATTN4_STAMP(tm5);
+
+        const int e_q0 = qb0, e_qw0 = qw0, e_tw = tw;
+        const bool more = q0n >= 0;
+        if (more) {
+            ATTN4_BLOCK_ISSUE(q0n);
+            q0n = -1;
+            seam = true;
+        }
+        int le_ = lane;
+        asm volatile("" : "+v"(le_));
+        const int c = le_ & 31, hi = le_ >> 5;
+        unsigned char* so = smem + STAGE + wave * TILE;
+#pragma unroll
+        for (int qb_ = 0; qb_ < 2; ++qb_) {
+            const int qg = e_qw0 + qb_ * 32 + c;
+            const bool valid = qg < seqlen && e_tw >= 0;
+            const float l_run = half_swap_sum((LS[qb_][0] + LS[qb_][1]) + (LS[qb_][2] + LS[qb_][3]));
+            const float inv = (valid && l_run > 0.f) ? 1.0f / l_run : 0.f;
+#pragma unroll
+            for (int db_ = 0; db_ < 4; ++db_) {
+                float x_[16];
+#include ATTN4_INC(epi_read.inc)
+#pragma unroll
+                for (int i4 = 0; i4 < 4; ++i4) {
+                    u32x2 w;
+                    w.x = pack2bf(x_[4 * i4 + 0] * inv, x_[4 * i4 + 1] * inv);
+                    w.y = pack2bf(x_[4 * i4 + 2] * inv, x_[4 * i4 + 3] * inv);
+                    *(u32x2*)(so + (qb_ * 32 + c) * 256 + (((db_ * 4 + i4) ^ (c & 15)) << 4) + hi * 8) = w;
+                }
+            }
+            float nm0;
+            if (qb_ == 0) asm volatile("v_mov_b32 %0, v192" : "=v"(nm0)); else asm volatile("v_mov_b32 %0, v208" : "=v"(nm0));
+            if (hi == 0 && qg < L) lse_base[qg] = valid ? (log2f(l_run) - nm0 * sl2) * 0.6931471805599453f : 0.f;
+        }
+        asm volatile("s_waitcnt lgkmcnt(0)\n\ts_barrier" ::: "memory");
+#pragma unroll
+        for (int k = 0; k < 16; ++k) {
+            const int r = 4 * k + (le_ >> 4), j = le_ & 15;
+            const int qg = e_qw0 + r;
+            if (qg < L) *(u32x4*)(o_base + (int64_t)qg * a.ld_o + j * 8) = *(const u32x4*)(so + r * 256 + ((j ^ (r & 15)) << 4));
+        }
+        if (a.dbg && le_ == 0) a.dbg[(((int64_t)b * a.Hq + hq) * nb + (e_q0 >> 8)) * 4 + wave] = nresc_;
+#ifdef MM355_ATTN4_TIMING
+        if (!more) {
+            asm volatile("s_waitcnt vmcnt(0)" ::: "memory");
+            const long long tm6 = __builtin_readcyclecounter();
+            if (le_ == 0 && (wave == 0 || wave == 3) && e_q0 + 64 <= L) {
+                long long* w = (long long*)(lse_base + e_q0) + (wave == 3 ? 8 : 0);
+                w[0] = tm1 - tm0; w[1] = tm2 - tm1; w[2] = tm3 - tm2; w[3] = tm4 - tm3; w[4] = tm5 - tm4; w[5] = tm6 - tm5; w[6] = e_tw; w[7] = T;
+            }
+        }
+        tm0 = __builtin_readcyclecounter();
+#endif
+        if (!more) break;
     }
-#pragma unroll
-    for (int ks = 0; ks < 8; ++ks) asm volatile("" : "+v"(KA[ks]));
-#pragma unroll
-    for (int i = 0; i < 4; ++i) { asm volatile("" : "+v"(VA[i])); asm volatile("" : "+v"(kvo[i])); asm volatile("" : "+v"(vvo[i])); }
-    int lim2[2] = {0, 0};
-    if (tw >= 0) {
-#pragma unroll
-        for (int qb = 0; qb < 2; ++qb) {
-            const int qg = qw0 + qb * 32 + c;
-            lim2[qb] = (a.causal ? min(qg, seqlen - 1) : seqlen - 1) - tw * 64 - 4 * hi;
-        }
+#undef ATTN4_BLOCK_ISSUE
+#undef ATTN4_PIECE_OFFSETS
+}
+
+}
+
+int mm355_attn4_fwd_launch(const attn2::Args& a, int variant, hipStream_t s) {
+    static std::atomic<uint64_t> ok_f{0}, ok_fs{0};
+    if (variant < 0 || variant > 5) return MM355_EINVAL;
+    const int64_t nb = (a.L + 255) / 256;
+    const int paired = (variant & 4) ? 1 : ((variant & 2) ? 0 : (a.causal && nb >= 2));
+    const int64_t nblk = (paired ? (nb + 1) / 2 : nb) * a.Hq * a.B;
+    if (nblk > 0x7fffffff) return MM355_EINVAL;
+    if (variant & 1) {
+        if (mm_ensure_dynamic_lds((const void*)attn4::fwd_kernel<true>, attn4::FWD_LDS, ok_fs) != MM355_OK) return MM355_ELAUNCH;
+        hipLaunchKernelGGL(attn4::fwd_kernel<true>, dim3((unsigned)nblk), dim3(256), attn4::FWD_LDS, s, a, paired);
+    } else {
+        if (mm_ensure_dynamic_lds((const void*)attn4::fwd_kernel<false>, attn4::FWD_LDS, ok_f) != MM355_OK) return MM355_ELAUNCH;
+        hipLaunchKernelGGL(attn4::fwd_kernel<false>, dim3((unsigned)nblk), dim3(256), attn4::FWD_LDS, s, a, paired);
     }
-    asm volatile("s_waitcnt vmcnt(12)" ::: "memory");
-#include ATTN4_INC(q_pre01.inc)
-    asm volatile("s_waitcnt vmcnt(0)" ::: "memory");
-    __builtin_amdgcn_s_barrier();
-
-#define ATTN4_STEP_VARS(s_) do { const int s__ = (s_); \
-    rsK = ATTN4_TILE_RSRC(kbase, s__ + 2); rsV = ATTN4_TILE_RSRC(vbase, s__ + 2); \
-    kdst = (s__ & 1) * TILE + wave * 4096; vdst = VRING + (s__ & 1) * TILE + wave * 4096; } while (0)
-
-    ATTN4_STAMP(tm1);
-    if (tw >= 0) {
-        bool mask_next = tw == 0;
-        ATTN4_STEP_VARS(-1);
-        if constexpr (SAFE) {
-#include ATTN4_INC(safe_head.inc)
-        } else {
-#include ATTN4_INC(head.inc)
-        }
-        ATTN4_STAMP(tm2);
-        int t = 0;
-        for (;;) {
-            if (t >= tw) break;
-            mask_next = t + 1 == tw;
-            ATTN4_STEP_VARS(t);
-            if constexpr (SAFE) {
-#include ATTN4_INC(safe_loop0.inc)
-            } else {
-#include ATTN4_INC(loop0.inc)
-            }
-            ++t;
-            if (t >= tw) break;
-            mask_next = t + 1 == tw;
-            ATTN4_STEP_VARS(t);
-            if constexpr (SAFE) {
-#include ATTN4_INC(safe_loop1.inc)
-            } else {
-#include ATTN4_INC(loop1.inc)
-            }
-            ++t;
-        }
-        ATTN4_STAMP(tm3);
-        do_bar = tw <= T - 2;
-        ATTN4_STEP_VARS(tw);
-        if (tw & 1) {
-            if constexpr (SAFE) {
-#include ATTN4_INC(safe_tail1.inc)
-            } else {
-#include ATTN4_INC(tail1.inc)
-            }
-        } else {
-            if constexpr (SAFE) {
-#include ATTN4_INC(safe_tail0.inc)
-            } else {
-#include ATTN4_INC(tail0.inc)
-            }
-        }
-    }
-    ATTN4_STAMP(tm4);
-    do_bar = true;
-    for (int s = tw < 0 ? -1 : tw + 1; s <= T - 2; ++s) {
-        ATTN4_STEP_VARS(s);
-        if (s >= 0) {
-#pragma unroll
-            for (int i = 0; i < 4; ++i) { ATTN4_DMA_K(i); }
-        }
-        ATTN4_BARRIER();
-#pragma unroll
-        for (int i = 0; i < 4; ++i) { ATTN4_DMA_V(i); }
-    }
-    asm volatile("s_nop 15\n\ts_nop 15\n\ts_nop 15\n\ts_nop 15\n\ts_waitcnt vmcnt(0) lgkmcnt(0)" ::: "memory");
-    __syncthreads();
-    ATTN4_STAMP(tm5);
-
-    unsigned char* so = smem + wave * TILE;
-#pragma unroll
-    for (int qb_ = 0; qb_ < 2; ++qb_) {
-        const int qg = qw0 + qb_ * 32 + c;
-        const bool valid = qg < seqlen && tw >= 0;
-        const float l_run = half_swap_sum((LS[qb_][0] + LS[qb_][1]) + (LS[qb_][2] + LS[qb_][3]));
-        const float inv = (valid && l_run > 0.f) ? 1.0f / l_run : 0.f;
-#pragma unroll
-        for (int db_ = 0; db_ < 4; ++db_) {
-            float x_[16];
-#include ATTN4_INC(epi_read.inc)
-#pragma unroll
-            for (int i4 = 0; i4 < 4; ++i4) {
-                u32x2 w;
-                w.x = pack2bf(x_[4 * i4 + 0] * inv, x_[4 * i4 + 1] * inv);
-                w.y = pack2bf(x_[4 * i4 + 2] * inv, x_[4 * i4 + 3] * inv);
-                *(u32x2*)(so + (qb_ * 32 + c) * 256 + (((db_ * 4 + i4) ^ (c & 15)) << 4) + hi * 8) = w;
-            }
-        }
-        float nm0;
-        if (qb_ == 0) asm volatile("v_mov_b32 %0, v192" : "=v"(nm0)); else asm volatile("v_mov_b32 %0, v208" : "=v"(nm0));
-        if (hi == 0 && qg < L) lse_base[qg] = valid ? (log2f(l_run) - nm0 * sl2) * 0.6931471805599453f : 0.f;
-    }
-    __syncthreads();
-#pragma unroll
-    for (int k = 0; k < 16; ++k) {
-        const int r = 4 * k + (lane >> 4), j = lane & 15;
-        const int qg = qw0 + r;
-        if (qg < L) *(u32x4*)(o_base + (int64_t)qg * a.ld_o + j * 8) = *(const u32x4*)(so + r * 256 + ((j ^ (r & 15)) << 4));
-    }
-    if (a.dbg && lane == 0) a.dbg[(((int64_t)b * a.Hq + hq) * ((L + 255) / 256) + xb) * 4 + wave] = nresc_;
-#ifdef MM355_ATTN4_TIMING
-    asm volatile("s_waitcnt vmcnt(0)" ::: "memory");
-    const long long tm6 = __builtin_readcyclecounter();
-    if (lane == 0 && (wave == 0 || wave == 3) && q0 + 64 <= L) {
-        long long* w = (long long*)(lse_base + q0) + (wave == 3 ? 8 : 0);
-        w[0] = tm1 - tm0; w[1] = tm2 - tm1; w[2] = tm3 - tm2; w[3] = tm4 - tm3; w[4] = tm5 - tm4; w[5] = tm6 - tm5; w[6] = tw; w[7] = T;
-    }
-#endif
-}
-
-}
-
-int mm355_attn4_fwd_launch(const attn2::Args& a, int variant, hipStream_t s) {
-    const int64_t nblk = (int64_t)((a.L + 255) / 256) * a.Hq * a.B;
-    if (nblk > 0x7fffffff) return MM355_EINVAL;
-    if (variant == 1) hipLaunchKernelGGL(attn4::fwd_kernel<true>, dim3((unsigned)nblk), dim3(256), 0, s, a);
-    else hipLaunchKernelGGL(attn4::fwd_kernel<false>, dim3((unsigned)nblk), dim3(256), 0, s, a);
     return mm_launch_status();
 }
diff --git a/metamorph_amd/csrc/attn4_bwd.hip b/metamorph_amd/csrc/attn4_bwd.hip
--- a/metamorph_amd/csrc/attn4_bwd.hip
+++ b/metamorph_amd/csrc/attn4_bwd.hip
@@ -302,61 +302,48 @@
 #endif
 }
 
+MM_DEV void q_pers_load(const uint16_t* p0_, const uint16_t* p1_) {
+#include ATTN4B_INC(q_pers_load.inc)
+}
 template <bool SAFE>
-__global__ __launch_bounds__(256, 1) __attribute__((amdgpu_num_vgpr(80))) void dq_kernel(Args a) {
+__global__ __launch_bounds__(256, 1) __attribute__((amdgpu_num_vgpr(80))) void dq_kernel(Args a, int paired) {
     extern __shared__ __attribute__((aligned(16))) unsigned char smem[];
     asm volatile("" ::: "v255", "a255");
     constexpr int NDMA = 8;
     const int tid = threadIdx.x, lane = tid & 63;
     const int wave = __builtin_amdgcn_readfirstlane(tid >> 6);
-    const int c = lane & 31, hi = lane >> 5;
+    const int nb = (a.L + 127) / 128;
     int xb, hq, b;
-    block_coords((a.L + 127) / 128, a.Hq, inner_heads(a.Hq, a.Hq / a.Hkv), true, xb, hq, b);
-    const int q0 = xb * 128;
+    block_coords(paired ? (nb + 1) / 2 : nb, a.Hq, inner_heads(a.Hq, a.Hq / a.Hkv), true, xb, hq, b);
     const int hk = hq / (a.Hq / a.Hkv);
     const int L = a.L;
     const int seqlen = a.seqlens ? min(a.seqlens[b], L) : L;
     const int64_t row_base = (int64_t)b * L;
     uint16_t* dq_base = a.dqb + row_base * a.ld_dq + (int64_t)hq * 128;
-    if (q0 >= seqlen) {
+    int q0 = (paired ? nb - 1 - xb : xb) * 128;
+    int q0n = (paired && nb - 1 - xb != xb) ? xb * 128 : -1;
+    while (q0 >= seqlen) {
         for (int v = tid; v < 128 * 16; v += 256) {
             const int r = v >> 4, cc = (v & 15) * 8;
             if (q0 + r < L) *(u32x4*)(dq_base + (int64_t)(q0 + r) * a.ld_dq + cc) = u32x4{0u, 0u, 0u, 0u};
         }
-        return;
-    }
-    const int kv_end = a.causal ? min(seqlen, q0 + 128) : seqlen;
-    const int n_tot = (kv_end + 63) >> 6;
-    const int qw0 = q0 + 32 * wave;
-    const int qg = qw0 + c;
+        if (q0n < 0) return;
+        q0 = q0n; q0n = -1;
+    }
     const uint32_t ldb = (uint32_t)a.ld_k * 2u;
     const uint16_t* kbase = a.k + row_base * a.ld_k + (int64_t)hk * 128;
     const uint16_t* vbase = a.v + row_base * a.ld_k + (int64_t)hk * 128;
     const uint32_t nrec = (uint32_t)(seqlen - 1) * ldb + 256u;
+    const int rpos = a.rope_pos ? __builtin_amdgcn_readfirstlane(a.rope_pos[b]) : 0;
 
     const uint32_t sl2b_ = __builtin_amdgcn_readfirstlane(__float_as_uint(a.scale * LOG2E));
-    LaneAddr la;
-    la.init(lane);
-    int RA[8], TA[4], TB[4], RAH[8], TAH[4], TBH[4];
-#pragma unroll
-    for (int i = 0; i < 8; ++i) { RA[i] = la.RA[i]; RAH[i] = RA[i] + 65536; asm volatile("" : "+v"(RA[i])); asm volatile("" : "+v"(RAH[i])); }
-#pragma unroll
-    for (int i = 0; i < 4; ++i) {
-        TA[i] = la.TA[i]; TB[i] = la.TB[i]; TAH[i] = TA[i] + 65536; TBH[i] = TB[i] + 65536;
-        asm volatile("" : "+v"(TA[i])); asm volatile("" : "+v"(TB[i])); asm volatile("" : "+v"(TAH[i])); asm volatile("" : "+v"(TBH[i]));
-    }
-    uint32_t kvo[4];
-    piece_offsets(wave, lane, ldb, kvo);
-#pragma unroll
-    for (int i = 0; i < 4; ++i) asm volatile("" : "+v"(kvo[i]));
     const float ninf = -INFINITY;
-    const int kmax = qg >= seqlen ? -1 : (a.causal ? min(qg, seqlen - 1) : seqlen - 1);
-    const int mlim_base = kmax - 4 * hi;
+    int n_tot, qw0, mlim_base, dt, ct;
     int mlim_ = 0;
     bool mask_cur = false;
 
     __amdgpu_buffer_rsrc_t rsK, rsV;
-    int dst0 = 0, dt = 0, ct = 0;
+    int dst0 = 0;
 #define Q_TILE_VARS(slot_) do { \
         rsK = __builtin_amdgcn_make_buffer_rsrc((void*)(kbase + (int64_t)dt * 64 * a.ld_k), 0, dt < n_tot ? nrec - (uint32_t)dt * 64u * ldb : 0u, 0x00020000); \
         rsV = __builtin_amdgcn_make_buffer_rsrc((void*)(vbase + (int64_t)dt * 64 * a.ld_k), 0, dt < n_tot ? nrec - (uint32_t)dt * 64u * ldb : 0u, 0x00020000); \
@@ -369,156 +356,221 @@
         const int kt0_ = ct * 64; \
         mask_cur = (a.causal && kt0_ + 63 > qw0) || kt0_ + 64 > seqlen || qw0 + 32 > seqlen; \
         mlim_ = mlim_base - kt0_; ++ct; } while (0)
-
-    Q_TILE_VARS(0);
-#pragma unroll
-    for (int i = 0; i < 8; ++i) { BWD_DMA(i); }
-    Q_TILE_VARS(1);
-#pragma unroll
-    for (int i = 0; i < 8; ++i) { BWD_DMA(i); }
-    {
-        const int qc = min(qg, L - 1);
-        const uint16_t* p0_ = a.q + (row_base + qc) * a.ld_q + (int64_t)hq * 128 + hi * 8;
-        const uint16_t* p1_ = a.d_o + (row_base + qc) * a.ld_o + (int64_t)hq * 128 + hi * 8;
-#include ATTN4B_INC(q_pers_load.inc)
-        const float nl_ = -a.lse_in[((int64_t)b * a.Hq + hq) * L + qc] * (1.0f / a.scale);
-        const float nd_ = -a.delta[((int64_t)b * a.Hq + hq) * L + qc];
+#define Q_BLOCK_ISSUE(q0_) do { \
+        const int q0__ = (q0_); \
+        int li_ = lane; \
+        asm volatile("" : "+v"(li_)); \
+        uint32_t kvo[4]; \
+        piece_offsets(wave, li_, ldb, kvo); \
+        const int kv_end_ = a.causal ? min(seqlen, q0__ + 128) : seqlen; \
+        n_tot = (kv_end_ + 63) >> 6; \
+        qw0 = q0__ + 32 * wave; \
+        const int qg = qw0 + (li_ & 31); \
+        const int kmax_ = qg >= seqlen ? -1 : (a.causal ? min(qg, seqlen - 1) : seqlen - 1);       \
+        mlim_base = kmax_ - 4 * (li_ >> 5); \
+        dt = 0; ct = 0; \
+        Q_TILE_VARS(0); \
+        _Pragma("unroll") for (int i = 0; i < 8; ++i) { BWD_DMA(i); } \
+        Q_TILE_VARS(1); \
+        _Pragma("unroll") for (int i = 0; i < 8; ++i) { BWD_DMA(i); } \
+        const int qc_ = min(qg, L - 1); \
+        const uint16_t* p0_ = a.q + (row_base + qc_) * a.ld_q + (int64_t)hq * 128 + (li_ >> 5) * 8; \
+        const uint16_t* p1_ = a.d_o + (row_base + qc_) * a.ld_o + (int64_t)hq * 128 + (li_ >> 5) * 8; \
+        q_pers_load(p0_, p1_); \
+        const float* pl_ = a.lse_in + ((int64_t)b * a.Hq + hq) * L + qc_; \
+        const float* pd_ = a.delta + ((int64_t)b * a.Hq + hq) * L + qc_; \
+        asm volatile("global_load_dword v224, %0, off\n\tglobal_load_dword v240, %1, off" :: "v"(pl_), "v"(pd_) : "memory"); \
+        if (a.rope_cos) { \
+            const uint16_t* pc_ = a.rope_cos + (int64_t)(qc_ + rpos) * 128 + 4 * (li_ >> 5); \
+            const uint16_t* ps_ = a.rope_sin + (int64_t)(qc_ + rpos) * 128 + 4 * (li_ >> 5); \
+            asm volatile(Q_ROPE_LOAD(192) :: "v"(pc_) : "memory"); \
+            asm volatile(Q_ROPE_LOAD(208) :: "v"(ps_) : "memory"); \
+        } } while (0)
+#define Q_ROPE_LOAD(r) "global_load_dwordx2 a[" #r ":" #r "+1], %0, off offset:0\n\tglobal_load_dwordx2 a[" #r "+2:" #r "+3], %0, off offset:16\n\t" \
+        "global_load_dwordx2 a[" #r "+4:" #r "+5], %0, off offset:32\n\tglobal_load_dwordx2 a[" #r "+6:" #r "+7], %0, off offset:48\n\t" \
+        "global_load_dwordx2 a[" #r "+8:" #r "+9], %0, off offset:64\n\tglobal_load_dwordx2 a[" #r "+10:" #r "+11], %0, off offset:80\n\t" \
+        "global_load_dwordx2 a[" #r "+12:" #r "+13], %0, off offset:96\n\tglobal_load_dwordx2 a[" #r "+14:" #r "+15], %0, off offset:112"
+#define Q_ROPE_READ(w_, r) asm volatile("v_accvgpr_read_b32 %0, a[" #r "]\n\tv_accvgpr_read_b32 %1, a[" #r "+1]" : "=v"((w_).x), "=v"((w_).y))
+
+    Q_BLOCK_ISSUE(q0);
+    for (;;) {
+        int ln_ = lane;
+        asm volatile("" : "+v"(ln_));
+        LaneAddr la;
+        la.init(ln_);
+        int RA[8], TA[4], TB[4], RAH[8], TAH[4], TBH[4];
+#pragma unroll
+        for (int i = 0; i < 8; ++i) { RA[i] = la.RA[i]; RAH[i] = RA[i] + 65536; asm volatile("" : "+v"(RA[i])); asm volatile("" : "+v"(RAH[i])); }
+#pragma unroll
+        for (int i = 0; i < 4; ++i) {
+            TA[i] = la.TA[i]; TB[i] = la.TB[i]; TAH[i] = TA[i] + 65536; TBH[i] = TB[i] + 65536;
+            asm volatile("" : "+v"(TA[i])); asm volatile("" : "+v"(TB[i])); asm volatile("" : "+v"(TAH[i])); asm volatile("" : "+v"(TBH[i]));
+        }
+        uint32_t kvo[4];
+        piece_offsets(wave, ln_, ldb, kvo);
+#pragma unroll
+        for (int i = 0; i < 4; ++i) asm volatile("" : "+v"(kvo[i]));
+#include ATTN4B_INC(q_zero.inc)
+        asm volatile("s_waitcnt vmcnt(0)" ::: "memory");
+        {
+            float lse_, del_;
+            asm volatile("v_mov_b32 %0, v224\n\tv_mov_b32 %1, v240" : "=v"(lse_), "=v"(del_));
+            const float nl_ = -lse_ * (1.0f / a.scale);
+            const float nd_ = -del_;
 #include ATTN4B_INC(q_tuple_write.inc)
-    }
-#include ATTN4B_INC(q_zero.inc)
-    asm volatile("s_waitcnt vmcnt(0)" ::: "memory");
-    {
-        float t0_, t1_;
+        }
+        {
+            float t0_, t1_;
 #include ATTN4B_INC(q_pers_place.inc)
-    }
-    __builtin_amdgcn_s_barrier();
-
-    Q_TILE_VARS(2);
-    if constexpr (SAFE) {
+        }
+        __builtin_amdgcn_s_barrier();
+
+        Q_TILE_VARS(2);
+        if constexpr (SAFE) {
 #include ATTN4B_INC(q_safe_head.inc)
-    } else {
+        } else {
 #include ATTN4B_INC(q_head.inc)
-    }
-    int u = 0;
-    for (;;) {
-        if (u >= n_tot - 1) break;
-        Q_TILE_VARS(3); Q_MASK_VARS();
-        if constexpr (SAFE) {
+        }
+        int u = 0;
+        for (;;) {
+            if (u >= n_tot - 1) break;
+            Q_TILE_VARS(3); Q_MASK_VARS();
+            if constexpr (SAFE) {
 #include ATTN4B_INC(q_safe_loop0.inc)
-        } else {
+            } else {
 #include ATTN4B_INC(q_loop0.inc)
-        }
-        ++u;
-        if (u >= n_tot - 1) break;
-        Q_TILE_VARS(0); Q_MASK_VARS();
-        if constexpr (SAFE) {
+            }
+            ++u;
+            if (u >= n_tot - 1) break;
+            Q_TILE_VARS(0); Q_MASK_VARS();
+            if constexpr (SAFE) {
 #include ATTN4B_INC(q_safe_loop1.inc)
-        } else {
+            } else {
 #include ATTN4B_INC(q_loop1.inc)
-        }
-        ++u;
-        if (u >= n_tot - 1) break;
-        Q_TILE_VARS(1); Q_MASK_VARS();
-        if constexpr (SAFE) {
+            }
+            ++u;
+            if (u >= n_tot - 1) break;
+            Q_TILE_VARS(1); Q_MASK_VARS();
+            if constexpr (SAFE) {
 #include ATTN4B_INC(q_safe_loop2.inc)
-        } else {
+            } else {
 #include ATTN4B_INC(q_loop2.inc)
-        }
-        ++u;
-        if (u >= n_tot - 1) break;
-        Q_TILE_VARS(2); Q_MASK_VARS();
-        if constexpr (SAFE) {
+            }
+            ++u;
+            if (u >= n_tot - 1) break;
+            Q_TILE_VARS(2); Q_MASK_VARS();
+            if constexpr (SAFE) {
 #include ATTN4B_INC(q_safe_loop3.inc)
-        } else {
+            } else {
 #include ATTN4B_INC(q_loop3.inc)
-        }
-        ++u;
-    }
-    Q_MASK_VARS();
-    switch (u & 3) {
-    case 0:
-        if constexpr (SAFE) {
+            }
+            ++u;
+        }
+        Q_MASK_VARS();
+        switch (u & 3) {
+        case 0:
+            if constexpr (SAFE) {
 #include ATTN4B_INC(q_safe_tail0.inc)
-        } else {
+            } else {
 #include ATTN4B_INC(q_tail0.inc)
-        }
-        break;
-    case 1:
-        if constexpr (SAFE) {
+            }
+            break;
+        case 1:
+            if constexpr (SAFE) {
 #include ATTN4B_INC(q_safe_tail1.inc)
-        } else {
+            } else {
 #include ATTN4B_INC(q_tail1.inc)
-        }
-        break;
-    case 2:
-        if constexpr (SAFE) {
+            }
+            break;
+        case 2:
+            if constexpr (SAFE) {
 #include ATTN4B_INC(q_safe_tail2.inc)
-        } else {
+            } else {
 #include ATTN4B_INC(q_tail2.inc)
-        }
-        break;
-    default:
-        if constexpr (SAFE) {
+            }
+            break;
+        default:
+            if constexpr (SAFE) {
 #include ATTN4B_INC(q_safe_tail3.inc)
-        } else {
+            } else {
 #include ATTN4B_INC(q_tail3.inc)
-        }
-        break;
+            }
+            break;
+        }
+        asm volatile("s_nop 15\n\ts_nop 15\n\ts_nop 15\n\ts_nop 15\n\ts_waitcnt vmcnt(0) lgkmcnt(0)" ::: "memory");
+        __syncthreads();
+
+        const int e_qw0 = qw0;
+        u32x2 cw[8], sw[8];
+#pragma unroll
+        for (int i = 0; i < 8; ++i) cw[i] = sw[i] = u32x2{0u, 0u};
+        if (a.rope_cos) {
+            Q_ROPE_READ(cw[0], 192); Q_ROPE_READ(cw[1], 194); Q_ROPE_READ(cw[2], 196); Q_ROPE_READ(cw[3], 198);
+            Q_ROPE_READ(cw[4], 200); Q_ROPE_READ(cw[5], 202); Q_ROPE_READ(cw[6], 204); Q_ROPE_READ(cw[7], 206);
+            Q_ROPE_READ(sw[0], 208); Q_ROPE_READ(sw[1], 210); Q_ROPE_READ(sw[2], 212); Q_ROPE_READ(sw[3], 214);
+            Q_ROPE_READ(sw[4], 216); Q_ROPE_READ(sw[5], 218); Q_ROPE_READ(sw[6], 220); Q_ROPE_READ(sw[7], 222);
+        }
+        const bool more = q0n >= 0;
+        if (more) {
+            Q_BLOCK_ISSUE(q0n);
+            q0n = -1;
+        }
+        int le_ = lane;
+        asm volatile("" : "+v"(le_));
+        const int ec = le_ & 31, ehi = le_ >> 5, e_qg = e_qw0 + ec;
+        unsigned char* so = smem + 3 * SLOT + wave * 8192;
+        const float keep = e_qg < seqlen ? a.scale : 0.0f;
+#pragma unroll
+        for (int dbp = 0; dbp < 2; ++dbp)
+#pragma unroll
+            for (int i4_ = 0; i4_ < 4; ++i4_) {
+                constexpr int which_ = 0;
+                float x_[4], lo_[4], hi_[4];
+                {
+                    const int db_ = dbp;
+#include ATTN4B_INC(q_acc_read.inc)
+#pragma unroll
+                    for (int r = 0; r < 4; ++r) lo_[r] = x_[r] * keep;
+                }
+                {
+                    const int db_ = dbp + 2;
+#include ATTN4B_INC(q_acc_read.inc)
+#pragma unroll
+                    for (int r = 0; r < 4; ++r) hi_[r] = x_[r] * keep;
+                }
+                if (a.rope_cos) {
+                    const u32x2 cw_ = cw[dbp * 4 + i4_], sw_ = sw[dbp * 4 + i4_];
+                    const float cs[4] = {bflo(cw_.x), bfhi(cw_.x), bflo(cw_.y), bfhi(cw_.y)};
+                    const float sn[4] = {bflo(sw_.x), bfhi(sw_.x), bflo(sw_.y), bfhi(sw_.y)};
+#pragma unroll
+                    for (int r = 0; r < 4; ++r) {
+                        const float x1 = round_bf(lo_[r]), x2 = round_bf(hi_[r]);
+                        lo_[r] = x1 * cs[r] + x2 * sn[r];
+                        hi_[r] = x2 * cs[r] - x1 * sn[r];
+                    }
+                }
+#pragma unroll
+                for (int half = 0; half < 2; ++half) {
+                    const int db = dbp + 2 * half;
+                    const float* s4 = half ? hi_ : lo_;
+                    u32x2 w;
+                    w.x = pack2bf(s4[0], s4[1]);
+                    w.y = pack2bf(s4[2], s4[3]);
+                    *(u32x2*)(so + ec * 256 + (((db * 4 + i4_) ^ (ec & 15)) << 4) + ehi * 8) = w;
+                }
+            }
+        asm volatile("s_waitcnt lgkmcnt(0)\n\ts_barrier" ::: "memory");
+#pragma unroll
+        for (int k = 0; k < 8; ++k) {
+            const int r = 4 * k + (le_ >> 4), j = le_ & 15;
+            if (e_qw0 + r < L) *(u32x4*)(dq_base + (int64_t)(e_qw0 + r) * a.ld_dq + j * 8) = *(const u32x4*)(so + r * 256 + ((j ^ (r & 15)) << 4));
+        }
+        if (!more) break;
     }
 #undef BWD_DMA
-    asm volatile("s_nop 15\n\ts_nop 15\n\ts_nop 15\n\ts_nop 15\n\ts_waitcnt vmcnt(0) lgkmcnt(0)" ::: "memory");
-    __syncthreads();
-
-    unsigned char* so = smem + wave * 8192;
-    const float keep = qg < seqlen ? a.scale : 0.0f;
-    const int pos = min(qg, L - 1) + (a.rope_pos ? a.rope_pos[b] : 0);
-#pragma unroll
-    for (int dbp = 0; dbp < 2; ++dbp)
-#pragma unroll
-        for (int i4_ = 0; i4_ < 4; ++i4_) {
-            constexpr int which_ = 0;
-            float x_[4], lo_[4], hi_[4];
-            {
-                const int db_ = dbp;
-#include ATTN4B_INC(q_acc_read.inc)
-#pragma unroll
-                for (int r = 0; r < 4; ++r) lo_[r] = x_[r] * keep;
-            }
-            {
-                const int db_ = dbp + 2;
-#include ATTN4B_INC(q_acc_read.inc)
-#pragma unroll
-                for (int r = 0; r < 4; ++r) hi_[r] = x_[r] * keep;
-            }
-            if (a.rope_cos) {
-                const int col = dbp * 32 + 8 * i4_ + 4 * hi;
-                const u32x2 cw = *(const u32x2*)(a.rope_cos + (int64_t)pos * 128 + col);
-                const u32x2 sw = *(const u32x2*)(a.rope_sin + (int64_t)pos * 128 + col);
-                const float cs[4] = {bflo(cw.x), bfhi(cw.x), bflo(cw.y), bfhi(cw.y)};
-                const float sn[4] = {bflo(sw.x), bfhi(sw.x), bflo(sw.y), bfhi(sw.y)};
-#pragma unroll
-                for (int r = 0; r < 4; ++r) {
-                    const float x1 = round_bf(lo_[r]), x2 = round_bf(hi_[r]);
-                    lo_[r] = x1 * cs[r] + x2 * sn[r];
-                    hi_[r] = x2 * cs[r] - x1 * sn[r];
-                }
-            }
-#pragma unroll
-            for (int half = 0; half < 2; ++half) {
-                const int db = dbp + 2 * half;
-                const float* s4 = half ? hi_ : lo_;
-                u32x2 w;
-                w.x = pack2bf(s4[0], s4[1]);
-                w.y = pack2bf(s4[2], s4[3]);
-                *(u32x2*)(so + c * 256 + (((db * 4 + i4_) ^ (c & 15)) << 4) + hi * 8) = w;
-            }
-        }
-    __syncthreads();
-#pragma unroll
-    for (int k = 0; k < 8; ++k) {
-        const int r = 4 * k + (lane >> 4), j = lane & 15;
-        if (qw0 + r < L) *(u32x4*)(dq_base + (int64_t)(qw0 + r) * a.ld_dq + j * 8) = *(const u32x4*)(so + r * 256 + ((j ^ (r & 15)) << 4));
-    }
+#undef Q_BLOCK_ISSUE
+#undef Q_ROPE_LOAD
+#undef Q_ROPE_READ
 }
 
 __global__ __launch_bounds__(256) void nstat_kernel(const float* __restrict__ lse, const float* __restrict__ delta, float* __restrict__ nstat, int64_t n,
@@ -533,20 +585,23 @@
 
 int mm355_attn4_bwd_launch(const attn2::Args& a, float* workspace, int variant, hipStream_t s) {
     static std::atomic<uint64_t> ok_kv{0}, ok_kvs{0}, ok_q{0}, ok_qs{0};
+    if (variant < 0 || variant > 5) return MM355_EINVAL;
     const int64_t n = (int64_t)a.B * a.Hq * a.L;
     hipLaunchKernelGGL(attn4b::nstat_kernel, dim3((unsigned)std::min<int64_t>((n + 255) / 256, 2048)), dim3(256), 0, s, a.lse_in, a.delta, workspace, n, 1.0f / a.scale);
-    const int64_t nkv = (int64_t)((a.L + 127) / 128) * a.Hkv * a.B, nq = (int64_t)((a.L + 127) / 128) * a.Hq * a.B;
+    const int64_t nb = (a.L + 127) / 128;
+    const int paired = (variant & 4) ? 1 : ((variant & 2) ? 0 : (a.causal && nb >= 2));
+    const int64_t nkv = nb * a.Hkv * a.B, nq = (paired ? (nb + 1) / 2 : nb) * a.Hq * a.B;
     if (nkv > 0x7fffffff || nq > 0x7fffffff) return MM355_EINVAL;
-    if (variant == 1) {
+    if (variant & 1) {
         if (mm_ensure_dynamic_lds((const void*)attn4b::dkdv_kernel<true>, attn4b::KV_LDS, ok_kvs) != MM355_OK) return MM355_ELAUNCH;
         if (mm_ensure_dynamic_lds((const void*)attn4b::dq_kernel<true>, attn4b::Q_LDS, ok_qs) != MM355_OK) return MM355_ELAUNCH;
         hipLaunchKernelGGL(attn4b::dkdv_kernel<true>, dim3((unsigned)nkv), dim3(256), attn4b::KV_LDS, s, a, (const float*)workspace);
-        hipLaunchKernelGGL(attn4b::dq_kernel<true>, dim3((unsigned)nq), dim3(256), attn4b::Q_LDS, s, a);
+        hipLaunchKernelGGL(attn4b::dq_kernel<true>, dim3((unsigned)nq), dim3(256), attn4b::Q_LDS, s, a, paired);
     } else {
         if (mm_ensure_dynamic_lds((const void*)attn4b::dkdv_kernel<false>, attn4b::KV_LDS, ok_kv) != MM355_OK) return MM355_ELAUNCH;
         if (mm_ensure_dynamic_lds((const void*)attn4b::dq_kernel<false>, attn4b::Q_LDS, ok_q) != MM355_OK) return MM355_ELAUNCH;
         hipLaunchKernelGGL(attn4b::dkdv_kernel<false>, dim3((unsigned)nkv), dim3(256), attn4b::KV_LDS, s, a, (const float*)workspace);
-        hipLaunchKernelGGL(attn4b::dq_kernel<false>, dim3((unsigned)nq), dim3(256), attn4b::Q_LDS, s, a);
+        hipLaunchKernelGGL(attn4b::dq_kernel<false>, dim3((unsigned)nq), dim3(256), attn4b::Q_LDS, s, a, paired);
     }
     return mm_launch_status();
 }
```
